# SolverForge/solverforge

Measured on AMD Instinct MI355X. Metric: moves-evaluated/sec, CVRP-1000 (nearby-list selector, LateAcceptance(400)+AcceptedCount(256)), higher is better.
Workload: dtype int64 score / int32 trial deltas (u16 matrix copy)

## Files before the change

solverforge_amd/csrc/sf_list_wave.hip:

```cpp
#pragma once
#include <hip/hip_runtime.h>
#include <stdint.h>

#include <type_traits>

#include "sf_list_model.h"

namespace sf {

constexpr uint32_t RC_MAX = 128;
constexpr uint32_t RC_SMALL = 64;
constexpr uint32_t NBR_NODE_MASK = 0x7FFFu;
constexpr uint32_t NBR_SAME_FLAG = 0x8000u;
constexpr uint32_t NBR_END = 0xFFFFu;
#ifndef SF_WPB
#define SF_WPB 4
#endif
constexpr int WPB = SF_WPB;

#ifndef SF_SPEC_V
#define SF_SPEC_V(x) (x)
#endif
#ifndef SF_SPEC_DIM
#define SF_SPEC_DIM(x) (x)
#endif
#ifndef SF_SPEC_NCAP
#define SF_SPEC_NCAP(x) (x)
#endif
#ifndef SF_SPEC_K0
#define SF_SPEC_K0(x) (x)
#endif
#ifndef SF_SPEC_K1
#define SF_SPEC_K1(x) (x)
#endif
#ifndef SF_SPEC_LA_SIZE
#define SF_SPEC_LA_SIZE(x) (x)
#endif
#ifndef SF_SPEC_LIMIT
#define SF_SPEC_LIMIT(x) (x)
#endif
#ifndef SF_SPEC_HAS_PERM
#define SF_SPEC_HAS_PERM(x) (x)
#endif
#ifndef SF_SPEC_HAS_EXPLICIT
#define SF_SPEC_HAS_EXPLICIT(x) (x)
#endif
#ifdef SF_SPEC_L
#define SF_SPEC_OWN_LANE(v) asm volatile("" : "+v"(v))
#else
#define SF_SPEC_OWN_LANE(v)
#endif
#ifdef SF_SPEC_NO_WIDE
#define SF_SPEC_WIDE_TIES(x) false
#else
#define SF_SPEC_WIDE_TIES(x) (x)
#endif
#ifdef SF_SPEC_NO_TIES
#define SF_SPEC_TIES(x) 0ULL
#else
#define SF_SPEC_TIES(x) (x)
#endif
#ifdef SF_SPEC_ROWS_FULL
#define SF_SPEC_ROW_HAVE(x) true
#define SF_SPEC_ROW_HAVEMASK(x) (~0ULL)
#else
#define SF_SPEC_ROW_HAVE(x) (x)
#define SF_SPEC_ROW_HAVEMASK(x) (x)
#endif


__device__ __forceinline__ void wave_sync() {
    __builtin_amdgcn_fence(__ATOMIC_RELEASE, "wavefront");
    __builtin_amdgcn_wave_barrier();
    __builtin_amdgcn_fence(__ATOMIC_ACQUIRE, "wavefront");
}

SF_PLAIN_KERNEL
__global__ __launch_bounds__(256) void k_nbr_presort(const int64_t* __restrict__ mat, int dim, int P,
                                                     uint16_t* __restrict__ keys) {
    extern __shared__ __attribute__((aligned(16))) unsigned char smem[];
    uint64_t* sk = (uint64_t*)smem;
    const int row = blockIdx.x;
    const int64_t* rp = mat + (size_t)row * dim;
    for (int t = threadIdx.x; t < P; t += blockDim.x) {
        uint64_t k = ~0ULL;
        if (t < dim) {
            const int64_t v = rp[t];
            if (v >= 0 && v != UNREACHABLE) k = ((uint64_t)v << 24) | (uint64_t)(uint32_t)t;
        }
        sk[t] = k;
    }
    __syncthreads();
    for (int size = 2; size <= P; size <<= 1)
        for (int stride = size >> 1; stride > 0; stride >>= 1) {
            for (int t = threadIdx.x; t < (P >> 1); t += blockDim.x) {
                const int lo = (t / stride) * 2 * stride + (t % stride);
                const int hi = lo + stride;
                const bool up = (lo & size) == 0;
                const uint64_t a = sk[lo], b = sk[hi];
                if ((a > b) == up) {
                    sk[lo] = b;
                    sk[hi] = a;
                }
            }
            __syncthreads();
        }
    for (int t = threadIdx.x; t < dim; t += blockDim.x) {
        const uint64_t k = sk[t];
        uint32_t e = NBR_END;
        if (k != ~0ULL) {
            e = (uint32_t)k & NBR_NODE_MASK;
            if (t > 0 && (sk[t - 1] >> 24) == (k >> 24)) e |= NBR_SAME_FLAG;
        }
        keys[(size_t)row * dim + t] = (uint16_t)e;
    }
}

struct WCarve {
    size_t load, off, node, ring, visits, rtab, routeat, total;
    uint32_t rc;
    __host__ __device__ WCarve(int V, int n_cap, int dim, int max_k, bool compact = false, bool node_global = false) {
        rc = max_k <= 32 ? RC_SMALL : RC_MAX;
        size_t o = 0;
        load = o;
        o = align_up(o + (compact ? sizeof(int32_t) : sizeof(int64_t)) * V, 16);
        off = o;
        o = align_up(o + (node_global ? sizeof(uint16_t) : sizeof(uint32_t)) * (V + 1), 16);
        node = o;
        o = align_up(o + (node_global ? 0 : (compact ? sizeof(uint16_t) : sizeof(uint32_t)) * dim), 16);
        ring = o;
        o = align_up(o + sizeof(uint32_t) * 2 * rc * MAX_LEAVES, 16);
        visits = o;
        o = align_up(o + sizeof(uint16_t) * n_cap, 16);
        rtab = o;
        o = align_up(o + (node_global ? 0 : sizeof(uint32_t) * V * MAX_LEAVES), 16);
        routeat = o;
        o = align_up(o + (compact ? 0 : sizeof(uint16_t) * V * MAX_LEAVES), 16);
        total = o;
    }
};

template <bool COMPACT>
struct NodeSlotT;
template <>
struct NodeSlotT<false> {
    uint32_t* p;
    __device__ __forceinline__ NodeSlotT(unsigned char* base, int, const uint16_t*, const void*, bool = false) : p((uint32_t*)base) {}
    __device__ __forceinline__ void clear(uint32_t node) const { p[node] = NODE_NONE; }
    __device__ __forceinline__ void set(uint32_t node, uint32_t route, uint32_t pos) const { p[node] = (route << 16) | pos; }
    __device__ __forceinline__ uint32_t get(uint32_t node) const { return p[node]; }
    __device__ __forceinline__ uint32_t word(uint32_t node) const { return p[node]; }
    __device__ __forceinline__ uint32_t wide(uint32_t s, uint32_t) const { return s; }
    __device__ __forceinline__ uint32_t wide_short(uint32_t s) const { return s; }
};
template <>
struct NodeSlotT<true> {
    uint16_t* p;
    const uint16_t* visits;
    const void* off;
    bool off16;
    uint32_t pb, pmax;
    __device__ __forceinline__ uint32_t off_at(uint32_t i) const { return off16 ? (uint32_t)((const uint16_t*)off)[i] : ((const uint32_t*)off)[i]; }
    __device__ __forceinline__ NodeSlotT(unsigned char* base, int V, const uint16_t* visits_, const void* off_, bool off16_ = false)
        : p((uint16_t*)base), visits(visits_), off(off_), off16(off16_) {
        uint32_t rb = 1;
        while ((1u << rb) - 1u < (uint32_t)V) ++rb;
        pb = 16u - rb;
        pmax = (1u << pb) - 1u;
    }
    __device__ __forceinline__ void clear(uint32_t node) const { p[node] = 0xFFFFu; }
    __device__ __forceinline__ void set(uint32_t node, uint32_t route, uint32_t pos) const {
        p[node] = (uint16_t)((route << pb) | (pos < pmax ? pos : pmax));
    }
    __device__ __forceinline__ uint32_t get(uint32_t node) const { return wide(p[node], node); }
    __device__ __forceinline__ uint32_t word(uint32_t node) const { return p[node]; }
    __device__ __forceinline__ uint32_t wide(uint32_t s, uint32_t node) const {
        const bool none = s == 0xFFFFu;
        const uint32_t route = s >> pb;
        uint32_t pos = s & pmax;
        if (__ballot(!none && pos == pmax) != 0ull) {
            if (!none && pos == pmax) {
                const uint32_t o = off_at(route), len = off_at(route + 1) - o;
                while (pos + 1 < len && (uint32_t)visits[o + pos] != node) ++pos;
            }
        }
        return none ? NODE_NONE : ((route << 16) | pos);
    }
    __device__ __forceinline__ uint32_t wide_short(uint32_t s) const {
        const uint32_t w = ((s >> pb) << 16) | (s & pmax);
        return s == 0xFFFFu ? NODE_NONE : w;
    }
};
__host__ __device__ inline bool node_slot_compact_ok(int V) { return V >= 1 && V <= 1022; }

struct NearbyItem {
    uint32_t w;
    uint32_t ord;
    uint32_t pay0;
    uint32_t pay1;
};

__device__ __forceinline__ NearbyItem nearby_item(bool is_change, uint32_t slot, uint32_t se, uint32_t sp,
                                                  uint32_t len, uint32_t k, const uint32_t* s_off,
                                                  const uint16_t* sb, const uint16_t* ro) {
    const bool some = slot != NODE_NONE;
    const uint32_t r2 = some ? slot >> 16 : 0u, dp = slot & 0xFFFFu;
    const uint32_t len2 = s_off[r2 + 1] - s_off[r2];
    const uint32_t rk = ro[r2];
    const uint32_t inter_ord = ORD_INTER_BASE + (uint32_t)sb[rk] + dp;
    const bool intra = r2 == se;
    const uint32_t end_pay = (r2 << 16) | len2;
    NearbyItem it;
    if (is_change) {
        const bool v0 = !intra || (dp != sp && dp != sp + 1);
        const bool v1 = dp + 1 == len2 && (!intra || len != sp + 1);
        it.w = some ? (uint32_t)v0 + (uint32_t)v1 : 0u;
        it.ord = intra ? (v0 ? dp : len) : inter_ord;
        it.pay0 = v0 ? slot : end_pay;
        it.pay1 = end_pay;
    } else {
        const bool v = intra ? dp > sp : rk > k;
        it.w = (some && v) ? 1u : 0u;
        it.ord = intra ? dp : inter_ord;
        it.pay0 = slot;
        it.pay1 = 0;
    }
    return it;
}

struct RouteTab {
    const uint32_t* rt;
    static constexpr int KEY_SHIFT = 24;
    __device__ __forceinline__ uint32_t word(uint32_t route) const { return rt[route]; }
    __device__ __forceinline__ static uint32_t rank(uint32_t w) { return w & 0xFFFFu; }
    __device__ __forceinline__ static uint32_t inter_ord(uint32_t w, uint32_t dp) { return ORD_INTER_BASE + (w >> 16) + dp; }
};
#ifdef SF_SPEC_TIE_KEY
static_assert(SF_SPEC_RB >= 1 && SF_SPEC_PB >= 1 && SF_SPEC_RB + SF_SPEC_PB <= 22, "SF_SPEC_TIE_KEY: the packed word does not fit 32 bits");
constexpr uint32_t ORD_ARITH_BASE = 1u << (SF_SPEC_RB + SF_SPEC_PB);
constexpr int ORD_ARITH_SHIFT = SF_SPEC_PB;
#else
constexpr uint32_t ORD_ARITH_BASE = 1u << 26;
constexpr int ORD_ARITH_SHIFT = 16;
#endif
struct RouteArith {
    uint32_t st, inv, V, recip;
    static constexpr int KEY_SHIFT = 28;
    __device__ __forceinline__ uint32_t word(uint32_t route) const {
        uint32_t x = route + V - st;
        x = x >= V ? x - V : x;
        const uint32_t y = x * inv;
        uint32_t rk = y - __umulhi(y, recip) * V;
        return rk >= V ? rk - V : rk;
    }
    __device__ __forceinline__ static uint32_t rank(uint32_t w) { return w; }
    __device__ __forceinline__ static uint32_t inter_ord(uint32_t w, uint32_t dp) { return ORD_ARITH_BASE + (w << ORD_ARITH_SHIFT) + dp; }
};
struct RouteRank {
    const uint32_t* rt;
    static constexpr int KEY_SHIFT = RouteArith::KEY_SHIFT;
    __device__ __forceinline__ uint32_t word(uint32_t route) const { return rt[route]; }
    __device__ __forceinline__ static uint32_t rank(uint32_t w) { return w; }
    __device__ __forceinline__ static uint32_t inter_ord(uint32_t w, uint32_t dp) { return RouteArith::inter_ord(w, dp); }
};
template <class OT, class RT>
__device__ __forceinline__ NearbyItem nearby_item_rt(bool is_change, uint32_t slot, uint32_t se, uint32_t sp,
                                                     uint32_t len, uint32_t k, const OT* s_off, const RT& rt) {
    const bool some = slot != NODE_NONE;
    const uint32_t r2 = some ? slot >> 16 : 0u, dp = slot & 0xFFFFu;
    const uint32_t len2 = s_off[r2 + 1] - s_off[r2];
    const uint32_t t = rt.word(r2);
    const uint32_t rk = RT::rank(t);
    const uint32_t inter_ord = RT::inter_ord(t, dp);
    const bool intra = r2 == se;
    const uint32_t end_pay = (r2 << 16) | len2;
    NearbyItem it;
    if (is_change) {
        const bool v0 = !intra || (dp != sp && dp != sp + 1);
        const bool v1 = dp + 1 == len2 && (!intra || len != sp + 1);
        it.w = some ? (uint32_t)v0 + (uint32_t)v1 : 0u;
        it.ord = intra ? (v0 ? dp : len) : inter_ord;
        it.pay0 = v0 ? slot : end_pay;
        it.pay1 = end_pay;
    } else {
        const bool v = intra ? dp > sp : rk > k;
        it.w = (some && v) ? 1u : 0u;
        it.ord = intra ? dp : inter_ord;
        it.pay0 = slot;
        it.pay1 = 0;
    }
    return it;
}

__device__ __forceinline__ uint32_t mbcnt64(uint64_t mask) {
    return __builtin_amdgcn_mbcnt_hi((uint32_t)(mask >> 32), __builtin_amdgcn_mbcnt_lo((uint32_t)mask, 0u));
}
#ifdef SF_SPEC_TIE_KEY
__device__ __forceinline__ int32_t tie_key_fix(uint64_t startmask, uint64_t nonstart, uint32_t ord, uint32_t wc) {
    const uint32_t q = (mbcnt64(startmask >> 1) << (SF_SPEC_RB + SF_SPEC_PB + 3)) | (ord << 2) | wc;
    uint32_t q_dn = q, q_up = q;
    int32_t fix = 0;
    uint64_t run = nonstart;
    for (uint32_t d = 1; run != 0; ++d) {
        q_dn = (uint32_t)__builtin_amdgcn_update_dpp(0, (int)q_dn, 0x130, 0xf, 0xf, true);
        q_up = (uint32_t)__builtin_amdgcn_update_dpp(0, (int)q_up, 0x138, 0xf, 0xf, true);
        fix += q_dn < q ? (int32_t)(q_dn & 3u) : 0;
        fix -= q_up > q ? (int32_t)(q_up & 3u) : 0;
        run &= nonstart << d;
    }
    return fix;
}
#endif

template <class LT, class OT, bool OWN_LANE = false>
__device__ __forceinline__ void apply_list_move_wave(const ListModel& m, uint16_t* visits, OT* off,
                                                     LT* load, int kind, uint32_t a, uint32_t i, uint32_t b,
                                                     uint32_t j, uint32_t ext = 0) {
    uint32_t lane = threadIdx.x & 63u;
    if constexpr (OWN_LANE) asm volatile("" : "+v"(lane));
    if (kind == 2) {
        const uint32_t P = off[a] + i, Q = off[b] + j;
        const uint32_t x = visits[P];
        wave_sync();
        if (P < Q) {
            for (uint32_t t0 = P; t0 < Q; t0 += 64) {
                const uint32_t t = t0 + lane;
                uint32_t nv = 0;
                if (t < Q) nv = (t + 1 < Q) ? (uint32_t)visits[t + 1] : x;
                wave_sync();
                if (t < Q) visits[t] = (uint16_t)nv;
                wave_sync();
            }
        } else if (P > Q) {
            for (uint32_t c0 = 0; c0 <= P - Q; c0 += 64) {
                const uint32_t dd = c0 + lane;
                const bool in = dd <= P - Q;
                const uint32_t t = P - (in ? dd : 0u);
                uint32_t nv = 0;
                if (in) nv = t > Q ? (uint32_t)visits[t - 1] : x;
                wave_sync();
                if (in) visits[t] = (uint16_t)nv;
                wave_sync();
            }
        }
        if (a != b) {
            for (uint32_t rr = lane; rr <= (uint32_t)SF_SPEC_V(m.V); rr += 64) {
                if (a < b && rr > a && rr <= b) off[rr] -= 1;
                if (a > b && rr > b && rr <= a) off[rr] += 1;
            }
            if (lane == 0 && m.demand) {
                const int64_t dx = (int64_t)m.demand[x];
                load[a] = (LT)wsub(load[a], dx);
                load[b] = (LT)wadd(load[b], dx);
            }
        }
    } else if (kind == 6) {
        const uint32_t za = ext & 0xFFFFu, zb = ext >> 16;
        const uint32_t PA = off[a] + i, PB = off[b] + j;
        const bool a_first = PA < PB;
        const uint32_t PX = a_first ? PA : PB, zx = a_first ? za : zb, PY = a_first ? PB : PA, zy = a_first ? zb : za;
        const uint32_t ox = a_first ? a : b, oy = a_first ? b : a;
        int64_t da = 0, db = 0;
        if (a != b && m.demand) {
            for (uint32_t t = 0; t < za; ++t) da = wadd(da, (int64_t)m.demand[visits[PA + t]]);
            for (uint32_t t = 0; t < zb; ++t) db = wadd(db, (int64_t)m.demand[visits[PB + t]]);
        }
        wave_sync();
        relocate_flat_segment(visits, PY, zy, PX, lane, 64u, [] { wave_sync(); });
        relocate_flat_segment(visits, PX + zy, zx, PY + zy, lane, 64u, [] { wave_sync(); });
        if (a != b) {
            for (uint32_t rr = lane; rr <= (uint32_t)SF_SPEC_V(m.V); rr += 64)
                if (rr > ox && rr <= oy) off[rr] = off[rr] + zy - zx;
            if (lane == 0 && m.demand) {
                load[a] = (LT)wadd(wsub(load[a], da), db);
                load[b] = (LT)wadd(wsub(load[b], db), da);
            }
        }
    } else if (kind == 5) {
        const uint32_t z = ext - i, P = off[a] + i;
        const uint32_t Q = a != b ? off[b] + j : (j <= i ? off[a] + j : off[a] + j + z);
        int64_t dsum = 0;
        if (a != b && m.demand)
            for (uint32_t t = 0; t < z; ++t) dsum = wadd(dsum, (int64_t)m.demand[visits[P + t]]);
        wave_sync();
        relocate_flat_segment(visits, P, z, Q, lane, 64u, [] { wave_sync(); });
        if (a != b) {
            for (uint32_t rr = lane; rr <= (uint32_t)SF_SPEC_V(m.V); rr += 64) {
                if (a < b && rr > a && rr <= b) off[rr] -= z;
                if (a > b && rr > b && rr <= a) off[rr] += z;
            }
            if (lane == 0 && m.demand) {
                load[a] = (LT)wsub(load[a], dsum);
                load[b] = (LT)wadd(load[b], dsum);
            }
        }
    } else if (kind == 4) {
        const uint32_t lo = off[a] + i, hi = off[a] + j;
        for (uint32_t t = lane; t < (hi - lo) / 2; t += 64) {
            const uint16_t x = visits[lo + t], y = visits[hi - 1 - t];
            visits[lo + t] = y;
            visits[hi - 1 - t] = x;
        }
    } else if (kind == 9) {
        const uint32_t base = off[a] + i, size = j - i;
        const uint32_t perm = nth_permutation_nibbles(size, ext);
        uint32_t nv = 0;
        if (lane < size) nv = visits[base + ((perm >> (4u * lane)) & 15u)];
        wave_sync();
        if (lane < size) visits[base + lane] = (uint16_t)nv;
    } else if (kind == 7) {
        const uint32_t base = off[a], c1 = i, c2 = b, c3 = j;
        const uint32_t mask = kopt_reverse_mask(ext);
        const bool rb = (mask >> 1) & 1u, rc = (mask >> 2) & 1u;
        auto reverse_range = [&](uint32_t lo, uint32_t hi) {
            for (uint32_t t = lane; t < (hi - lo) / 2; t += 64) {
                const uint16_t x = visits[base + lo + t], y = visits[base + hi - 1 - t];
                visits[base + lo + t] = y;
                visits[base + hi - 1 - t] = x;
            }
            wave_sync();
        };
        if (!kopt_swaps_segments(ext)) {
            if (rb) reverse_range(c1, c2);
            if (rc) reverse_range(c2, c3);
        } else {
            const uint32_t zc = c3 - c2;
            reverse_range(c1, c3);
            if (!rc) reverse_range(c1, c1 + zc);
            if (!rb) reverse_range(c1 + zc, c3);
        }
    } else if (kind == 3) {
        if (lane == 0) {
            const uint32_t pa = off[a] + i, pb = off[b] + j;
            const uint16_t x = visits[pa], y = visits[pb];
            visits[pa] = y;
            visits[pb] = x;
            if (a != b && m.demand) {
                const int64_t dx = (int64_t)m.demand[x], dy = (int64_t)m.demand[y];
                load[a] = (LT)wadd(wsub(load[a], dx), dy);
                load[b] = (LT)wadd(wsub(load[b], dy), dx);
            }
        }
    }
    wave_sync();
}

__device__ __forceinline__ uint32_t nearby_source_to_ring(const ListModel& m, const NbrIndex& nb, bool is_change, uint32_t se,
                                                          uint32_t sp, uint32_t len, uint32_t k, uint32_t sx,
                                                          const uint32_t* node_slot, const uint32_t* s_off, const uint16_t* sb,
                                                          const uint16_t* ro, uint32_t* rq, uint32_t RCM, uint32_t tl,
                                                          uint32_t key, uint32_t base, uint32_t need, uint32_t emitted) {
    const uint32_t lane = threadIdx.x & 63u;
    const uint64_t lanebit = 1ULL << lane;
    const uint32_t dim = (uint32_t)m.dim;
    const uint16_t* rowk = nb.keys + (size_t)sx * dim;
    const uint32_t mv0 = (se << 16) | sp;
    for (;;) {
        const bool have = key != NBR_END;
        const uint64_t havemask = __ballot(have);
        if (havemask == 0) break;
        NearbyItem it{0u, 0u, 0u, 0u};
        if (have) it = nearby_item(is_change, node_slot[key & NBR_NODE_MASK], se, sp, len, k, s_off, sb, ro);
        const uint64_t startmask = __ballot(have && (lane == 0 || !(key & NBR_SAME_FLAG)));
        const bool more = havemask == ~0ULL && base + 64 < dim;
        const uint32_t fo = 63u - (uint32_t)__clzll((unsigned long long)startmask);
        if (more && fo == 0) {
            TopK tk{~0ULL, 0u, ~0ULL};
            for (uint32_t b2 = base; b2 < dim; b2 += 64) {
                const uint32_t j2 = b2 + lane;
                const uint32_t ky = j2 < dim ? (uint32_t)rowk[j2] : NBR_END;
                NearbyItem i2{0u, 0u, 0u, 0u};
                uint64_t hk = 0;
                if (ky != NBR_END) {
                    const uint32_t y2 = ky & NBR_NODE_MASK;
                    i2 = nearby_item(is_change, node_slot[y2], se, sp, len, k, s_off, sb, ro);
                    hk = (uint64_t)m.mat[(size_t)sx * dim + y2] << 24;
                }
                if (!__ballot(ky != NBR_END)) break;
                topk_offer(tk, need, i2.w >= 1 ? (hk | i2.ord) : ~0ULL, i2.pay0);
                topk_offer(tk, need, i2.w == 2 ? (hk | (i2.ord + 1)) : ~0ULL, i2.pay1);
            }
            const uint32_t cnt = (uint32_t)__popcll(__ballot(lane < need && tk.key != ~0ULL));
            if (lane < cnt) {
                const uint32_t qi = (tl + emitted + lane) & RCM;
                rq[qi * 2] = mv0;
                rq[qi * 2 + 1] = tk.pay;
            }
            emitted += cnt;
            break;
        }
        const uint32_t nclosed = more ? fo : (uint32_t)__popcll(havemask);
        const uint64_t closedmask = nclosed >= 64 ? ~0ULL : ((1ULL << nclosed) - 1ULL);
        const bool closed = (closedmask & lanebit) != 0;
        const uint32_t wc = closed ? it.w : 0u;
        const uint64_t w1 = __ballot(wc == 1), w2 = __ballot(wc == 2);
        const uint32_t Wc = (uint32_t)__popcll(w1) + 2u * (uint32_t)__popcll(w2);
        if (Wc > 0) {
            int32_t pos = (int32_t)(mbcnt64(w1) + 2u * mbcnt64(w2));
            const uint64_t nonstart = ~startmask & closedmask;
            if (nonstart) {
                const uint32_t packed = (it.ord << 2) | wc;
                uint64_t run = nonstart;
                for (uint32_t d = 1; run != 0; ++d) {
                    const uint32_t p_dn = __shfl_down(packed, d), p_up = __shfl_up(packed, d);
                    const bool same_up = (run & lanebit) != 0;
                    const bool same_dn = ((run >> d) & lanebit) != 0;
                    if (same_dn && (p_dn >> 2) < it.ord) pos += (int32_t)(p_dn & 3u);
                    if (same_up && (p_up >> 2) > it.ord) pos -= (int32_t)(p_up & 3u);
                    run &= nonstart << d;
                }
            }
            if (wc >= 1 && (uint32_t)pos < need) {
                const uint32_t qi = (tl + emitted + (uint32_t)pos) & RCM;
                rq[qi * 2] = mv0;
                rq[qi * 2 + 1] = it.pay0;
            }
            if (wc == 2 && (uint32_t)pos + 1 < need) {
                const uint32_t qi = (tl + emitted + (uint32_t)pos + 1) & RCM;
                rq[qi * 2] = mv0;
                rq[qi * 2 + 1] = it.pay1;
            }
            const uint32_t ne = Wc < need ? Wc : need;
            emitted += ne;
            need -= ne;
        }
        if (need == 0 || !more) break;
        base += nclosed;
        const uint32_t jj = base + lane;
        key = jj < dim ? (uint32_t)rowk[jj] : NBR_END;
    }
    return emitted;
}

#if defined(SF_PHASE_PROFILE) || defined(SF_GEN_COUNT)
__device__ unsigned long long g_phase[8];
#endif
#ifdef SF_ISA_MARK
#define ISA_MARK(name) asm volatile("; SF_MARK " name)
#else
#define ISA_MARK(name)
#endif
#if defined(SF_PHASE_PROFILE) && !defined(SF_PHASE_PGRP)
#define PH_DECL uint64_t ph_t = clock64(), ph_acc[8] = {0, 0, 0, 0, 0, 0, 0, 0};
#define PH(i)                          \
    {                                  \
        const uint64_t _t = clock64(); \
        ph_acc[i] += _t - ph_t;        \
        ph_t = _t;                     \
    }
#define PH_DUMP \
    if (lane == 0) for (int _k = 0; _k < 8; ++_k) atomicAdd(&g_phase[_k], (unsigned long long)ph_acc[_k]);
#elif defined(SF_GEN_COUNT)
#define PH_DECL uint64_t ph_acc[8] = {0, 0, 0, 0, 0, 0, 0, 0};
#define PH(i)
#define GC(i) ph_acc[i] += 1;
#define PH_DUMP \
    if (lane == 0) for (int _k = 0; _k < 8; ++_k) atomicAdd(&g_phase[_k], (unsigned long long)ph_acc[_k]);
#else
#define PH_DECL
#define PH(i)
#define PH_DUMP
#endif
#ifndef GC
#define GC(i)
#endif

__device__ __forceinline__ int32_t wave_max_i32(int32_t v) {
    const int lo = (int)0x80000000;
    v = max(v, __builtin_amdgcn_update_dpp(lo, v, 0x111, 0xf, 0xf, false));
    v = max(v, __builtin_amdgcn_update_dpp(lo, v, 0x112, 0xf, 0xf, false));
    v = max(v, __builtin_amdgcn_update_dpp(lo, v, 0x114, 0xf, 0xf, false));
    v = max(v, __builtin_amdgcn_update_dpp(lo, v, 0x118, 0xf, 0xf, false));
    v = max(v, __builtin_amdgcn_update_dpp(lo, v, 0x142, 0xa, 0xf, false));
    v = max(v, __builtin_amdgcn_update_dpp(lo, v, 0x143, 0xc, 0xf, false));
    return __builtin_amdgcn_readlane(v, 63);
}
template <int L>
__device__ __forceinline__ bool small_ge(const int32_t (&a)[L], const int32_t (&b)[L]) {
    bool ge = true;
#pragma unroll
    for (int k = L - 1; k >= 0; --k) ge = a[k] > b[k] || (a[k] == b[k] && ge);
    return ge;
}
template <int L>
__device__ __forceinline__ bool small_ge0(const int32_t (&a)[L]) {
    bool ge = true;
#pragma unroll
    for (int k = L - 1; k >= 0; --k) ge = a[k] > 0 || (a[k] == 0 && ge);
    return ge;
}
__device__ __forceinline__ int32_t clamp_i64_to_i32(int64_t v) {
    return v > 0x7FFFFFFFll ? 0x7FFFFFFF : v < -0x7FFFFFFFll - 1 ? (int32_t)0x80000000 : (int32_t)v;
}

template <int L, class LT, bool M16 = false, class OT = uint32_t>
__device__ __forceinline__ bool eval_list_move_small(const ListModel& m, const uint16_t* visits, const OT* off, const LT* load,
                                                     bool chg, uint32_t a, uint32_t i, uint32_t b, uint32_t j, int32_t (&dv)[L]) {
    const uint32_t oa = off[a], la = off[a + 1] - oa;
    const uint32_t ob = off[b], lb = off[b + 1] - ob;
    const bool intra = a == b;
    bool ok = i < la && (chg ? j <= lb : j < lb) && !(intra && (j == i || (chg && j == i + 1)));
    const bool flip = !chg && intra && i > j;
    const uint32_t i2 = ok ? (flip ? j : i) : 0u, j2 = ok ? (flip ? i : j) : 0u;
    const uint32_t la_ = ok ? la : 0u, lb_ = ok ? lb : 0u;
    const uint32_t depot = (uint32_t)m.depot;
    const uint32_t P = oa + i2, Q = ob + j2;
    const bool has_pa = i2 > 0, has_na = i2 + 1 < la_, has_q = j2 < lb_, has_pb = j2 > 0, has_nb = j2 + 1 < lb_;
    const uint32_t r_x = visits[P];
    const uint32_t x = ok ? r_x : depot;
    const uint32_t r_pa = visits[has_pa ? P - 1 : P], r_na = visits[has_na ? P + 1 : P];
    const uint32_t r_q = visits[has_q ? Q : P], r_pb = visits[has_pb ? Q - 1 : P], r_nb = visits[has_nb ? Q + 1 : P];
    const uint32_t pa = has_pa ? r_pa : depot, na = has_na ? r_na : depot;
    const uint32_t vq = has_q ? r_q : depot;
    const uint32_t pb = has_pb ? r_pb : depot, nb = has_nb ? r_nb : depot;
    ok = ok && (chg || x != vq);
    const bool adj = !chg && intra && j2 == i2 + 1;
    const bool ca = chg || adj;
    const bool src_single = la == 1, dst_empty = !intra && lb == 0;
    const uint32_t dim4 = (uint32_t)SF_SPEC_DIM(m.dim) * (M16 ? 2u : 4u);
    auto leg = [&](uint32_t f, uint32_t t) -> uint32_t {
        const uint32_t byte_off = f * dim4 + t * (M16 ? 2u : 4u);
        if (M16) return *(const uint16_t*)((const char*)m.mat16 + byte_off);
        return *(const uint32_t*)((const char*)m.mat32 + byte_off);
    };
    const uint32_t p0 = leg(pa, chg ? na : vq);
    const uint32_t p1 = leg(chg ? pb : vq, ca ? x : na);
    const uint32_t p2 = leg(ca ? x : pb, chg ? vq : (adj ? nb : x));
    const uint32_t p3 = leg(x, nb);
    const uint32_t m0 = leg(pa, x);
    const uint32_t m1 = leg(x, adj ? vq : na);
    const uint32_t m3 = leg(vq, nb);
    const uint32_t m2 = leg(adj ? vq : pb, adj ? nb : vq);
    int32_t d_cap = 0;
    if (m.cap_level >= 0) {
        const int32_t dx = m.demand[x];
        const int32_t dyq = m.demand[vq];
        const int32_t dy = chg ? 0 : dyq;
        const int32_t cap = (int32_t)m.capacity;
        const int32_t la0 = (int32_t)load[a], lb0 = (int32_t)load[b];
        const int32_t la1 = la0 - dx + dy, lb1 = lb0 - dy + dx;
        d_cap = max(la1 - cap, 0) + max(lb1 - cap, 0) - max(la0 - cap, 0) - max(lb0 - cap, 0);
        d_cap = intra ? 0 : d_cap;
    }
    const uint32_t plus = ((chg && src_single) ? 0u : p0) + p1 + p2 + (ca ? 0u : p3);
    const uint32_t minus = m0 + m1 + ((chg && dst_empty) ? 0u : m2) + (ca ? 0u : m3);
    const int32_t d_dist = (int32_t)(plus - minus);
    const int32_t cw = (int32_t)m.cap_weight, dw = (int32_t)m.dist_weight;
#pragma unroll
    for (int k = 0; k < L; ++k) {
        int32_t v = 0;
        if (k == m.cap_level) v -= cw * d_cap;
        if (k == m.dist_level) v -= dw * d_dist;
        dv[k] = ok ? v : 0;
    }
    return ok;
}

template <int L>
struct LevelWords {
    uint32_t wc[L], wd[L];
    uint32_t has_cap;
    int32_t cap, cw, dw;
    uint32_t depot;
};
template <int L, bool USED, bool KW>
__device__ __forceinline__ LevelWords<L> level_words(const ListModel& m) {
    LevelWords<L> w;
    w.cap = w.cw = w.dw = 0;
    w.depot = 0;
#ifdef SF_SPEC_MODEL_WORDS
    w.cap = SF_SPEC_CAPACITY, w.cw = SF_SPEC_CAP_WEIGHT, w.dw = SF_SPEC_DIST_WEIGHT, w.depot = SF_SPEC_DEPOT;
#pragma unroll
    for (int k = 0; k < L; ++k) w.wc[k] = k == SF_SPEC_CAP_LEVEL ? 0xFFFFFFFFu : 0u, w.wd[k] = k == SF_SPEC_DIST_LEVEL ? 0xFFFFFFFFu : 0u;
    w.has_cap = SF_SPEC_CAP_LEVEL >= 0 ? 1u : 0u;
    return w;
#endif
    if constexpr (KW) {
        auto word = [](uint32_t v) -> uint32_t {
            asm volatile("" : "+v"(v));
            return uni(v);
        };
        w.cap = (int32_t)word((uint32_t)m.capacity);
        w.cw = (int32_t)word((uint32_t)m.cap_weight);
        w.dw = (int32_t)word((uint32_t)m.dist_weight);
        w.depot = word((uint32_t)m.depot);
    }
#pragma unroll
    for (int k = 0; k < L; ++k) {
        w.wc[k] = uni(k == m.cap_level ? 0xFFFFFFFFu : 0u);
        w.wd[k] = uni(k == m.dist_level ? 0xFFFFFFFFu : 0u);
        if constexpr (USED) {
            asm volatile("" : "+s"(w.wc[k]));
            asm volatile("" : "+s"(w.wd[k]));
        }
    }
    w.has_cap = uni(m.cap_level >= 0 ? 1u : 0u);
    if constexpr (USED) asm volatile("" : "+s"(w.has_cap));
    return w;
}
template <int L, class LT, bool M16 = false, class OT = uint32_t, bool KW = false>
__device__ __forceinline__ void eval_generated_small(const ListModel& m, const LevelWords<L>& lw, const uint16_t* visits, const OT* off, const LT* load, uint32_t c,
                                                     uint32_t a, uint32_t i, uint32_t b, uint32_t j, int32_t (&dv)[L]) {
    const uint32_t oa = off[a], la = off[a + 1] - oa;
    const uint32_t ob = off[b], lb = off[b + 1] - ob;
    const uint32_t depot = KW ? lw.depot : (uint32_t)m.depot;
    const uint32_t P = oa + i, Q = ob + j;
    const uint32_t h_pa = min(i, 1u), h_na = min(la - 1u - i, 1u);
    const uint32_t h_q = min(lb - j, 1u), h_pb = min(j, 1u);
    const uint32_t h_nb = min(max(lb, j + 1u) - (j + 1u), 1u);
    const uint32_t x = visits[P];
    const uint32_t r_pa = visits[P - h_pa], r_na = visits[P + h_na];
    const uint32_t r_q = visits[Q - (1u - h_q)], r_pb = visits[Q - h_pb], r_nb = visits[Q + h_nb];
    const uint32_t pa = h_pa ? r_pa : depot, na = h_na ? r_na : depot;
    const uint32_t vq = h_q ? r_q : depot;
    const uint32_t pb = h_pb ? r_pb : depot, nb = h_nb ? r_nb : depot;
    const bool chg = c != 0;
    const bool intra = a == b;
    const bool adj = !chg && intra && j == i + 1;
    const bool ca = chg || adj;
    const uint32_t dim4 = (uint32_t)SF_SPEC_DIM(m.dim) * (M16 ? 2u : 4u);
    auto leg = [&](uint32_t f, uint32_t t) -> uint32_t {
        const uint32_t byte_off = __umul24(f, dim4) + t * (M16 ? 2u : 4u);
        if (M16) return *(const uint16_t*)((const char*)m.mat16 + byte_off);
        return *(const uint32_t*)((const char*)m.mat32 + byte_off);
    };
    const uint32_t p0 = leg(pa, chg ? na : vq);
    const uint32_t p1 = leg(chg ? pb : vq, ca ? x : na);
    const uint32_t p2 = leg(ca ? x : pb, chg ? vq : (adj ? nb : x));
    const uint32_t p3 = leg(x, nb);
    const uint32_t m0 = leg(pa, x);
    const uint32_t m1 = leg(x, adj ? vq : na);
    const uint32_t m3 = leg(vq, nb);
    const uint32_t m2 = leg(adj ? vq : pb, adj ? nb : vq);
    int32_t d_cap = 0;
    if (lw.has_cap != 0u) {
        const int32_t dx = m.demand[x];
        const int32_t dyq = m.demand[vq];
        const int32_t dy = chg ? 0 : dyq;
        const int32_t cap = KW ? lw.cap : (int32_t)m.capacity;
        const int32_t la0 = (int32_t)load[a] - cap, lb0 = (int32_t)load[b] - cap;
        const int32_t sh = dx - dy;
        d_cap = max(la0 - sh, 0) + max(lb0 + sh, 0) - max(la0, 0) - max(lb0, 0);
        d_cap = intra ? 0 : d_cap;
    }
    const uint32_t plus = ((chg && la == 1) ? 0u : p0) + p1 + p2 + (ca ? 0u : p3);
    const uint32_t minus = m0 + m1 + ((chg && !intra && lb == 0) ? 0u : m2) + (ca ? 0u : m3);
    const int32_t d_dist = (int32_t)(plus - minus);
    const int32_t tc = -((KW ? lw.cw : (int32_t)m.cap_weight) * d_cap), td = -((KW ? lw.dw : (int32_t)m.dist_weight) * d_dist);
#pragma unroll
    for (int k = 0; k < L; ++k) dv[k] = (int32_t)(((uint32_t)tc & lw.wc[k]) + ((uint32_t)td & lw.wd[k]));
}

struct LeafCursor {
    uint32_t head, tail;
    uint32_t left;
    uint32_t k, o;
    uint32_t se, len, sp, sx;
    uint32_t vk, vbase;
    int ex;
    uint32_t pk;
    uint32_t pv;
    uint32_t cend;
};

struct WaveArgs {
    ListModel m;
    SearchParams p;
    NbrIndex nb;
};
typedef const __attribute__((address_space(4))) WaveArgs* ColdArgs;
__device__ __forceinline__ ColdArgs cold_args() {
    uint64_t u = (uint64_t)__builtin_amdgcn_kernarg_segment_ptr();
    asm volatile("" : "+s"(u));
    return (ColdArgs)u;
}

#ifndef SF_WAVES_PER_EU
#define SF_WAVES_PER_EU 4
#endif
template <int L, bool TRACE, int MODE, bool COMPACT = false, int WPE = SF_WAVES_PER_EU, bool NODEG = false>
__global__ __launch_bounds__(64 * WPB, WPE) void k_list_search_wave(ListModel m, SearchParams p, NbrIndex nb) {
    constexpr bool FAST = MODE >= 1, SMALL = MODE == 2;
    constexpr bool LEAN = FAST && SMALL;
    constexpr bool SAT = LEAN && COMPACT, RANKTAB = LEAN && COMPACT && !NODEG;
    constexpr bool RBATCH = LEAN && !NODEG;
#define SF_COLD_P(f) (SMALL ? cold_args()->p.f : p.f)
#define SF_COLD_M(f) (SMALL ? cold_args()->m.f : m.f)
    static_assert(!COMPACT || SMALL, "COMPACT stores loads in 32 bits: MODE 2 only");
    static_assert(!NODEG || COMPACT, "NODEG: the 16-bit table of the COMPACT layout");
    using LT = typename std::conditional<COMPACT, int32_t, int64_t>::type;
    using OT = typename std::conditional<NODEG, uint16_t, uint32_t>::type;
    extern __shared__ __attribute__((aligned(16))) unsigned char smem[];
    const uint32_t lane = threadIdx.x & 63u;
    const uint32_t wave_in_group = uni(threadIdx.x >> 6);
    const int rr = (int)(blockIdx.x * (blockDim.x >> 6) + wave_in_group);
    if (rr >= p.n_launch) return;
    const int r = rr + p.replica_base;
    const int V = SF_SPEC_V(m.V);
    const uint32_t dim = (uint32_t)SF_SPEC_DIM(m.dim);

    const int n_leaves = FAST ? 2 : p.n_leaves;
    const uint32_t K0 = (uint32_t)SF_SPEC_K0(p.leaf[0].max_nearby), K1 = n_leaves > 1 ? (uint32_t)SF_SPEC_K1(p.leaf[1].max_nearby) : 1u;
    const bool chg0 = FAST ? true : p.leaf[0].kind == 16, chg1 = FAST ? false : (n_leaves > 1 && p.leaf[1].kind == 16);
    const int acceptor = FAST ? 1 : p.acceptor, forager = FAST ? 0 : p.forager;
    const bool dry_run = FAST ? false : p.dry_run != 0;
    __shared__ uint64_t s_sa[FAST ? 1 : WPB][FAST ? 1 : SA_WORDS];
    uint64_t* saw = s_sa[FAST ? 0 : wave_in_group];
    const bool annealing = !FAST && acceptor == 3;
    if constexpr (!FAST)
        if (annealing) sa_load(saw, p.sa, r, lane);
    const int32_t desc0_w = p.leaf[0].descriptor, desc1_w = n_leaves > 1 ? p.leaf[1].descriptor : 0;
    const uint64_t desc0_q = SMALL ? 0 : (uint64_t)p.leaf[0].descriptor, desc1_q = (!SMALL && n_leaves > 1) ? (uint64_t)p.leaf[1].descriptor : 0;
    auto desc0 = [&]() -> uint64_t { return SMALL ? (uint64_t)(int64_t)desc0_w : desc0_q; };
    auto desc1 = [&]() -> uint64_t { return SMALL ? (uint64_t)(int64_t)desc1_w : desc1_q; };

    const WCarve cv(V, SF_SPEC_NCAP(m.n_cap), (int)dim, (int)(K0 > K1 ? K0 : K1), COMPACT, NODEG);
    const uint32_t RCM = cv.rc - 1;
    unsigned char* mem = smem + (size_t)wave_in_group * cv.total;
    LT* s_load = (LT*)(mem + cv.load);
    OT* s_off = (OT*)(mem + cv.off);
    uint32_t* ring = (uint32_t*)(mem + cv.ring);
    uint16_t* s_visits = (uint16_t*)(mem + cv.visits);
    const NodeSlotT<COMPACT> node_slot(NODEG ? (unsigned char*)(m.node_tab + (size_t)r * dim) : mem + cv.node, V, s_visits, (const void*)s_off, NODEG);
    auto node_sync = [&]() {
        if constexpr (NODEG) {
            __builtin_amdgcn_fence(__ATOMIC_RELEASE, "workgroup");
            __builtin_amdgcn_wave_barrier();
            __builtin_amdgcn_fence(__ATOMIC_ACQUIRE, "workgroup");
        } else {
            wave_sync();
        }
    };
    constexpr bool ARANK = NODEG;
    using RT = typename std::conditional<ARANK, RouteArith, typename std::conditional<RANKTAB, RouteRank, RouteTab>::type>::type;
    uint32_t* rtab = (uint32_t*)(mem + cv.rtab);
    uint16_t* route_at = (uint16_t*)(mem + cv.routeat);

    uint32_t* g_visits = m.visits + (size_t)r * SF_SPEC_NCAP(m.n_cap);
    uint32_t* g_off = m.off + (size_t)r * (V + 1);
    int64_t* g_load = m.load + (size_t)r * V;
    int64_t* g_score = m.score + (size_t)r * 4;
    const bool tracing = TRACE && r == p.trace_replica;

    for (uint32_t t = lane; t <= (uint32_t)V; t += 64) s_off[t] = (OT)g_off[t];
    for (uint32_t t = lane; t < (uint32_t)V; t += 64) s_load[t] = (LT)g_load[t];
    for (uint32_t t = lane; t < dim; t += 64) node_slot.clear(t);
    node_sync();
    const uint32_t total0 = uni(s_off[V]);
    if (COMPACT && SF_SPEC_HAS_PERM(m.perm != nullptr)) {
        for (uint32_t t = lane; t < total0; t += 64) s_visits[t] = m.perm[g_visits[t]];
    } else {
        for (uint32_t t = lane; t < total0; t += 64) s_visits[t] = (uint16_t)g_visits[t];
    }
    wave_sync();
    for (uint32_t v = lane; v < (uint32_t)V; v += 64) {
        const uint32_t o = s_off[v], len = s_off[v + 1] - o;
        for (uint32_t q = 0; q < len; ++q) node_slot.set(s_visits[o + q], v, q);
    }
    node_sync();

    uint32_t nsat = 0;
    if constexpr (SAT) {
        for (uint32_t base = 0; base < (uint32_t)V; base += 64) {
            const uint32_t v = base + lane;
            const bool lg = v < (uint32_t)V && (uint32_t)(s_off[v + 1] - s_off[v]) > node_slot.pmax;
            nsat += (uint32_t)__popcll(__ballot(lg));
        }
    }
    auto ext_id = [&](uint32_t x) -> uint32_t { return (COMPACT && SF_SPEC_HAS_PERM(m.inv != nullptr)) ? (uint32_t)m.inv[x] : x; };
    int64_t cur[L], best_sol[L];
#pragma unroll
    for (int k = 0; k < L; ++k) {
        cur[k] = (int64_t)uni64((uint64_t)g_score[k]);
        best_sol[k] = (int64_t)uni64((uint64_t)m.best_score[(size_t)r * 4 + k]);
    }
    uint32_t st_steps = 0, st_gen = 0, st_acc = 0, st_applied = 0, st_calc = 0, st_scored = 0, st_sources = 0;
    uint64_t steps_run = 0;
    auto flush_stats = [&]() {
        if (lane == 0) {
            uint64_t* gs = SF_COLD_P(stats) + (size_t)r * SF_STATS_WORDS;
            gs[0] += st_steps;
            gs[1] += st_gen;
            gs[2] += st_gen;
            gs[3] += st_acc;
            gs[4] += st_applied;
            gs[5] += st_calc;
            gs[6] += st_gen - st_calc;
            gs[7] += st_scored;
            gs[8] += st_sources;
        }
        if constexpr (!SMALL) steps_run += st_steps;
        st_steps = st_gen = st_acc = st_applied = st_calc = st_scored = st_sources = 0;
    };
    uint64_t trace_n = 0;
    const uint64_t step_index0 = dry_run ? 0 : p.step_index[r];
    const uint64_t seed_draws0 = dry_run ? 0 : p.seed_draws[r];
    const int la_idx0 = dry_run ? 0 : p.la_idx[r];
    int la_cursor = la_idx0;
    const uint64_t lanebit = 1ULL << lane;
    uint32_t hm = 0;
    if constexpr (LEAN) {
        hm = (uint32_t)((int32_t)(lane << 26) >> 31);
        asm volatile("" : "+v"(hm));
    }
    auto half = [&](uint32_t lo, uint32_t up) -> uint32_t { return (lo & ~hm) | (up & hm); };
    PH_DECL

    const LevelWords<L> lvl = level_words<L, SMALL, RBATCH>(m);
    bool best_pending = false;
    const FastMod fm_V = make_fastmod(V > 0 ? (uint32_t)V : 1u);
    const FastMod fm_V1 = make_fastmod(V > 1 ? (uint32_t)V - 1u : 1u);
    const uint32_t v_recip32 = V > 1 ? (uint32_t)(0x100000000ull / (uint32_t)V) : 0u;
    const bool use_cm = V >= 2 && V <= 128;
    const uint64_t cm_lo = use_cm ? __ballot(lane >= 1 && lane < (uint32_t)V && gcd_u32(lane, (uint32_t)V) == 1) : 0ull;
    const uint64_t cm_hi = use_cm ? __ballot(lane + 64 < (uint32_t)V && gcd_u32(lane + 64, (uint32_t)V) == 1) : 0ull;
    int64_t step = 0;
    for (; step < SF_COLD_P(n_steps); ++step) {
        PH(7)
        ISA_MARK("prologue_begin");
        uint64_t sidx, sseed;
        if (dry_run) {
            sidx = p.dry_step_index;
            sseed = p.dry_step_seed;
        } else {
            sidx = step_index0 + (uint64_t)step;
            const uint64_t draw = seed_draws0 + (uint64_t)step;
            const uint64_t* const explicit_seeds = SF_COLD_P(explicit_seeds);
            const int64_t n_explicit = SF_COLD_P(n_explicit);
            if (SF_SPEC_HAS_EXPLICIT(explicit_seeds != nullptr) && (int64_t)draw < n_explicit)
                sseed = explicit_seeds[(size_t)r * n_explicit + draw];
            else
                sseed = step_seed(SF_COLD_P(random_seed) + (uint64_t)r, draw);
        }
        sidx = uni64(sidx);
        sseed = uni64(sseed);
        const StreamCtx ctx{sidx, sseed, FAST ? 3 : p.order};
        ScoreV<L> late;
#pragma unroll
        for (int k = 0; k < L; ++k) late.v[k] = 0;
        const int la_slot = la_cursor;
        if (acceptor == 1 || acceptor == 4) {
            const int64_t* const lh = SF_COLD_P(la_hist) + ((size_t)r * SF_SPEC_LA_SIZE(SF_COLD_P(la_size)) + la_slot) * 4;
#pragma unroll
            for (int k = 0; k < L; ++k) late.v[k] = (int64_t)uni64((uint64_t)lh[k]);
        }
        ScoreV<L> dla_thr = late;
        if (acceptor == 4) {
            ScoreV<L> db;
#pragma unroll
            for (int k = 0; k < L; ++k) db.v[k] = (int64_t)uni64((uint64_t)p.dla_best[(size_t)r * 4 + k]);
            dla_thr = dla_threshold<L>(db, p.dla_tolerance);
        }
        [[maybe_unused]] bool thr_on = true;
        if constexpr (TRACE)
            if (acceptor == 5 || acceptor == 6) ax_step_begin<L>(acceptor, p.sa.state + (size_t)r * SA_WORDS, late, thr_on);
        [[maybe_unused]] TabuStep<L> tabu;
        [[maybe_unused]] const TabuScope tabu_scope{0u, 0u, 0u};
        if constexpr (TRACE)
            if (acceptor == 7) tabu_step_begin<L>(p.sa.state + (size_t)r * SA_WORDS, tabu);
        int has_best = 0;
        typename std::conditional<SMALL, uint32_t, uint64_t>::type equal_count = 0;
        uint32_t accepted = 0, pulls = 0;
        ScoreV<L> best;
#pragma unroll
        for (int k = 0; k < L; ++k) best.v[k] = 0;
        uint32_t best_m0 = 0, best_m1 = 0;
        int best_leaf = 0;
        uint64_t best_ti = 0;
        int32_t late_d[L], best_d[L];
#pragma unroll
        for (int k = 0; k < L; ++k) {
            late_d[k] = SMALL ? clamp_i64_to_i32(wsub(late.v[k], cur[k])) : 0;
            best_d[k] = 0;
        }
        int64_t acc_thr = 0, best_key = 0;
        if constexpr (SMALL && L == 2) {
            const int64_t lh = late_d[0] < -(1 << 30) ? -(int64_t)(1 << 30) : (int64_t)late_d[0];
            const int64_t late_key = lh * 4294967296ll + (int64_t)late_d[1];
            acc_thr = late_key < 0 ? late_key : 0;
        }
        const uint32_t total = uni(s_off[V]);
        uint32_t hashed = 0;
        const bool lane_hash = FAST && use_cm;
        if (lane_hash) {
            const uint64_t es0 = SALT_NEARBY_CHANGE_ENTITY ^ desc0(), es1 = SALT_NEARBY_SWAP_ENTITY ^ desc1();
            const uint64_t salt = lane == 0 ? SALT_UNION_OFFSET : lane == 1 ? es0 : lane == 2 ? (es0 ^ STRIDE_SALT_MIX) : lane == 3 ? es1 : (es1 ^ STRIDE_SALT_MIX);
            const FastMod fm2 = make_fastmod(2u);
            FastMod f;
            f.M = lane == 0 ? fm2.M : ((lane & 1u) ? fm_V.M : fm_V1.M);
            f.n = lane == 0 ? fm2.n : ((lane & 1u) ? fm_V.n : fm_V1.n);
            hashed = fastmod_u64(ctx.mixed_seed(salt), f);
        }
        const uint32_t first_leaf = lane_hash ? (uint32_t)__builtin_amdgcn_readlane((int)hashed, 0)
                                              : (n_leaves > 1 ? ctx.random_index((uint32_t)n_leaves, SALT_UNION_OFFSET) : 0u);

        uint32_t perm_st0 = 0, perm_sd0 = 1, perm_st1 = 0, perm_sd1 = 1;
        uint32_t perm_inv0 = 0, perm_inv1 = 0;
        auto route_facts = [&](int l) -> RT {
            if constexpr (ARANK)
                return RouteArith{l ? perm_st1 : perm_st0, l ? perm_inv1 : perm_inv0, (uint32_t)V, v_recip32};
            else
                return RT{rtab + l * V};
        };
        auto resolve = [&](LeafCursor& c, int l) {
            const uint16_t* ra = route_at + l * V;
            uint32_t k = c.k, o = c.o, se = c.se, len = c.len;
            if (o >= c.cend) {
            ISA_MARK("resolve_slow_begin");
            if (k != c.vk || o >= len) {
                for (;;) {
                    if constexpr (COMPACT) {
                        const uint32_t xx = (l ? perm_st1 : perm_st0) + k * (l ? perm_sd1 : perm_sd0);
                        uint32_t rr_ = xx - __umulhi(xx, v_recip32) * (uint32_t)V;
                        rr_ = rr_ >= (uint32_t)V ? rr_ - (uint32_t)V : rr_;
                        se = uni(rr_);
                    } else
                        se = uni((uint32_t)ra[k]);
                    len = uni(s_off[se + 1] - s_off[se]);
                    if (o < len) break;
                    ++k;
                    o = 0;
                }
            }
            if (k != c.vk || (o & ~63u) != c.vbase) {
                const uint64_t src_salt = ((l ? chg1 : chg0) ? SALT_NEARBY_CHANGE_SOURCE : SALT_NEARBY_SWAP_SOURCE) ^
                                          (uint64_t)se ^ (l ? desc1() : desc0());
                const uint32_t oo = (o & ~63u) + lane;
                const uint32_t spl = oo < len ? ctx.selection_index(oo, len, src_salt) : 0u;
                const uint32_t sxl = oo < len ? (uint32_t)s_visits[s_off[se] + spl] : 0u;
                c.pv = spl | (sxl << 16);
                c.vk = k;
                c.vbase = o & ~63u;
            }
            c.cend = len < (o & ~63u) + 64u ? len : (o & ~63u) + 64u;
            c.k = k;
            c.se = se;
            c.len = len;
            ISA_MARK("resolve_slow_end");
            }
            const uint32_t pvv = (uint32_t)__builtin_amdgcn_readlane((int)c.pv, (int)(o & 63u));
            const uint32_t sp = pvv & 0xFFFFu, sx = pvv >> 16;
            c.o = o;
            c.sp = sp;
            c.sx = sx;
            const uint32_t ent = l ? ((lane + 32u) & 63u) : lane;
            const uint32_t entc = ent < dim ? ent : dim - 1u;
            const uint32_t pk_any = (uint32_t) * (const uint16_t*)((const char*)nb.keys + ((sx * dim + entc) << 1));
            if constexpr (LEAN)
                c.pk = pk_any;
            else
                c.pk = ent < dim ? pk_any : NBR_END;
        };
        auto row_key = [&](uint32_t raw, uint32_t e) -> uint32_t { return LEAN ? (e < dim ? raw : NBR_END) : raw; };

        PH(0)
        LeafCursor C0{0, 0, total, 0, 0, 0, 0, 0, 0, 0xFFFFFFFFu, 0, 0, NBR_END, 0, 0};
        LeafCursor C1{0, 0, n_leaves > 1 ? total : 0u, 0, 0, 0, 0, 0, 0, 0xFFFFFFFFu, 0, n_leaves > 1 ? 0 : 1, NBR_END, 0, 0};
        for (int l = 0; l < n_leaves; ++l) {
            const uint64_t ent_salt = ((l ? chg1 : chg0) ? SALT_NEARBY_CHANGE_ENTITY : SALT_NEARBY_SWAP_ENTITY) ^ (l ? desc1() : desc0());
            uint32_t pst, psd;
            if (lane_hash) {
                pst = (uint32_t)__builtin_amdgcn_readlane((int)hashed, l ? 3 : 1);
                psd = StreamCtx::first_coprime_from((uint32_t)__builtin_amdgcn_readlane((int)hashed, l ? 4 : 2) + 1u, cm_lo, cm_hi);
            } else if (use_cm)
                ctx.perm_params_fm(fm_V, fm_V1, ent_salt, pst, psd, cm_lo, cm_hi);
            else
                ctx.perm_params((uint32_t)V, ent_salt, pst, psd);
            pst = uni(pst);
            psd = uni(psd);
            if (l)
                perm_st1 = pst, perm_sd1 = psd;
            else
                perm_st0 = pst, perm_sd0 = psd;
            if constexpr (ARANK) {
                uint32_t inv = 0;
                for (uint32_t base = 0; base < (uint32_t)V; base += 64) {
                    const uint32_t c = base + lane;
                    const uint32_t xx = psd * c;
                    uint32_t rm = xx - __umulhi(xx, v_recip32) * (uint32_t)V;
                    rm = rm >= (uint32_t)V ? rm - (uint32_t)V : rm;
                    const uint64_t hit = __ballot(c < (uint32_t)V && rm == 1u);
                    if (hit) {
                        inv = base + (uint32_t)__ffsll((unsigned long long)hit) - 1u;
                        break;
                    }
                }
                if (l)
                    perm_inv1 = inv;
                else
                    perm_inv0 = inv;
                continue;
            }
            uint16_t* ra = route_at + l * V;
            uint32_t* rt = rtab + l * V;
            [[maybe_unused]] uint32_t carry = 0;
            for (uint32_t base = 0; base < (uint32_t)V; base += 64) {
                const uint32_t k = base + lane;
                if constexpr (RANKTAB) {
                    if (k < (uint32_t)V) rt[perm_index_recip(pst, psd, k, (uint32_t)V, v_recip32)] = k;
                } else {
                    uint32_t v = 0, e = 0;
                    if (k < (uint32_t)V) {
                        e = fastmod_u64((uint64_t)pst + (uint64_t)k * psd, fm_V);
                        if constexpr (!COMPACT) ra[k] = (uint16_t)e;
                        v = s_off[e + 1] - s_off[e] + 1;
                    }
                    const uint32_t inc = wave_incl_scan(v);
                    if (k < (uint32_t)V) rt[e] = k | ((carry + inc - v) << 16);
                    carry += __shfl(inc, 63);
                }
            }
        }
        wave_sync();
        if constexpr (SMALL) st_sources += C0.left + C1.left;
        if (total > 0) {
            resolve(C0, 0);
            if (n_leaves > 1) resolve(C1, 1);
        }
        ISA_MARK("prologue_end");

        PH(1)
        int done = 0;
        while (!done) {
            PH(4)
            auto gen_rest = [&](int l, uint32_t se, uint32_t sp, uint32_t len, uint32_t k, uint32_t sx, uint32_t tl,
                                uint32_t key, uint32_t base, uint32_t need, uint32_t emitted) -> uint32_t {
                const bool is_change = l ? chg1 : chg0;
                const RT rt = route_facts(l);
                uint32_t* rq = ring + (size_t)l * cv.rc * 2;
                const uint16_t* rowk = nb.keys + (size_t)sx * dim;
                const uint32_t mv0 = (se << 16) | sp;
                for (;;) {
                    const bool have = key != NBR_END;
                    const uint64_t havemask = __ballot(have);
                    if (havemask == 0) break;
                    NearbyItem it{0u, 0u, 0u, 0u};
                    if (have) it = nearby_item_rt(is_change, node_slot.get(key & NBR_NODE_MASK), se, sp, len, k, s_off, rt);
                    const uint64_t startmask = __ballot(have && (lane == 0 || !(key & NBR_SAME_FLAG)));
                    const bool more = havemask == ~0ULL && base + 64 < dim;
                    const uint32_t fo = 63u - (uint32_t)__clzll((unsigned long long)startmask);
                    if (SF_SPEC_WIDE_TIES(more && fo == 0)) {
                        TopK tk{~0ULL, 0u, ~0ULL};
                        for (uint32_t b2 = base; b2 < dim; b2 += 64) {
                            const uint32_t j2 = b2 + lane;
                            const uint32_t ky = j2 < dim ? (uint32_t)rowk[j2] : NBR_END;
                            NearbyItem i2{0u, 0u, 0u, 0u};
                            uint64_t hk = 0;
                            if (ky != NBR_END) {
                                const uint32_t y2 = ky & NBR_NODE_MASK;
                                i2 = nearby_item_rt(is_change, node_slot.get(y2), se, sp, len, k, s_off, rt);
                                hk = (uint64_t)m.mat[(size_t)ext_id(sx) * dim + ext_id(y2)] << RT::KEY_SHIFT;
                            }
                            if (!__ballot(ky != NBR_END)) break;
                            topk_offer(tk, need, i2.w >= 1 ? (hk | i2.ord) : ~0ULL, i2.pay0);
                            topk_offer(tk, need, i2.w == 2 ? (hk | (i2.ord + 1)) : ~0ULL, i2.pay1);
                        }
                        const uint32_t cnt = (uint32_t)__popcll(__ballot(lane < need && tk.key != ~0ULL));
                        if (lane < cnt) {
                            const uint32_t qi = (tl + emitted + lane) & RCM;
                            rq[qi * 2] = mv0;
                            rq[qi * 2 + 1] = tk.pay;
                        }
                        emitted += cnt;
                        break;
                    }
                    const uint32_t nclosed = more ? fo : (uint32_t)__popcll(havemask);
                    const uint64_t closedmask = nclosed >= 64 ? ~0ULL : ((1ULL << nclosed) - 1ULL);
                    const bool closed = (closedmask & lanebit) != 0;
                    const uint32_t wc = closed ? it.w : 0u;
                    const uint64_t w1 = __ballot(wc == 1), w2 = __ballot(wc == 2);
                    const uint32_t Wc = (uint32_t)__popcll(w1) + 2u * (uint32_t)__popcll(w2);
                    GC(l ? 6 : 5)
                    if (Wc == 0) { GC(7) }
                    if (Wc > 0) {
                        int32_t pos = (int32_t)(mbcnt64(w1) + 2u * mbcnt64(w2));
                        const uint64_t nonstart = SF_SPEC_TIES(~startmask & closedmask);
#ifdef SF_SPEC_TIE_KEY
                        if (nonstart) pos += tie_key_fix(startmask, nonstart, it.ord, wc);
#else
                        if (nonstart) {
                            const uint32_t packed = (it.ord << 2) | wc;
                            uint64_t run = nonstart;
                            uint32_t p_dn = packed, p_up = packed;
                            for (uint32_t d = 1; run != 0; ++d) {
                                p_dn = (uint32_t)__builtin_amdgcn_update_dpp(0, (int)p_dn, 0x130, 0xf, 0xf, false);
                                p_up = (uint32_t)__builtin_amdgcn_update_dpp(0, (int)p_up, 0x138, 0xf, 0xf, false);
                                const bool same_up = (run & lanebit) != 0;
                                const bool same_dn = ((run >> d) & lanebit) != 0;
                                if (same_dn && (p_dn >> 2) < it.ord) pos += (int32_t)(p_dn & 3u);
                                if (same_up && (p_up >> 2) > it.ord) pos -= (int32_t)(p_up & 3u);
                                run &= nonstart << d;
                            }
                        }
#endif
                        if (wc >= 1 && (uint32_t)pos < need) {
                            const uint32_t qi = (tl + emitted + (uint32_t)pos) & RCM;
                            rq[qi * 2] = mv0;
                            rq[qi * 2 + 1] = it.pay0;
                        }
                        if (wc == 2 && (uint32_t)pos + 1 < need) {
                            const uint32_t qi = (tl + emitted + (uint32_t)pos + 1) & RCM;
                            rq[qi * 2] = mv0;
                            rq[qi * 2 + 1] = it.pay1;
                        }
                        const uint32_t ne = Wc < need ? Wc : need;
                        emitted += ne;
                        need -= ne;
                    }
                    if (need == 0 || !more) break;
                    base += nclosed;
                    const uint32_t jj = base + lane;
                    key = jj < dim ? (uint32_t)rowk[jj] : NBR_END;
                }
                return emitted;
            };
            auto slot_of = [&](uint32_t word, uint32_t node) -> uint32_t {
                if constexpr (SAT) {
                    uint32_t ns = nsat;
                    asm volatile("" : "+s"(ns));
                    if (ns != 0) return node_slot.wide(word, node);
                    return node_slot.wide_short(word);
                } else
                    return node_slot.wide(word, node);
            };
            const uint32_t single0 = cv.rc - K0 < 64u ? cv.rc - K0 : 64u, single1 = cv.rc - K1 < 64u ? cv.rc - K1 : 64u;
            ISA_MARK("fill_begin");
            for (;;) {
                const bool both_live = !C0.ex && !C1.ex;
                const bool need0 = !C0.ex && C0.left > 0 && C0.tail - C0.head < (both_live ? 32u : single0);
                const bool need1 = n_leaves > 1 && !C1.ex && C1.left > 0 && C1.tail - C1.head < (both_live ? 32u : single1);
                if (!need0 && !need1) break;
                if (need0 && need1) {
                    ISA_MARK("pair_begin");
                    GC(0)
                    const bool hi = lane >= 32;
                    const uint32_t seA = C0.se, spA = C0.sp, lenA = C0.len, kA = C0.k, sxA = C0.sx, tlA = C0.tail;
                    const uint32_t seB = C1.se, spB = C1.sp, lenB = C1.len, kB = C1.k, sxB = C1.sx, tlB = C1.tail;
                    uint32_t l31 = lane & 31u;
                    if constexpr (LEAN) asm volatile("" : "+v"(l31));
                    const uint32_t key = LEAN ? (SF_SPEC_ROW_HAVE(false) ? half(C0.pk, C1.pk) : row_key(half(C0.pk, C1.pk), l31)) : (hi ? C1.pk : C0.pk);
                    const bool have = SF_SPEC_ROW_HAVE(key != NBR_END);
                    uint32_t nd = have ? (key & NBR_NODE_MASK) : 0u;
                    uint32_t slot_word = 0;
                    if constexpr (LEAN) {
                        asm volatile("" : "+v"(nd)::"memory");
                        slot_word = node_slot.word(nd);
                    }
                    C0.left -= 1;
                    C0.o += 1;
                    if (C0.left > 0) resolve(C0, 0);
                    C1.left -= 1;
                    C1.o += 1;
                    if (C1.left > 0) resolve(C1, 1);
                    if constexpr (!SMALL) st_sources += 2;
                    uint32_t slot_any;
                    if constexpr (LEAN)
                        slot_any = slot_of(slot_word, nd);
                    else
                        slot_any = node_slot.get(nd);
                    const uint32_t slot = have ? slot_any : NODE_NONE;
                    NearbyItem it{0u, 0u, 0u, 0u};
                    uint32_t mv0, tl, Kh, rq_off;
                    if constexpr (LEAN) {
                        const uint32_t sev = half(seA, seB), spv = half(spA, spB);
                        mv0 = (sev << 16) | spv;
                        tl = half(tlA, tlB);
                        Kh = half(K0, K1);
                        rq_off = hm & (cv.rc * 2u);
                        const bool some = slot != NODE_NONE;
                        const uint32_t r_any = slot >> 16, dp = slot & 0xFFFFu;
                        const uint32_t r2 = some ? r_any : 0u;
                        const uint32_t len2 = s_off[r2 + 1] - s_off[r2];
                        uint32_t t;
                        if constexpr (ARANK)
                            t = RouteArith{half(perm_st0, perm_st1), half(perm_inv0, perm_inv1), (uint32_t)V, v_recip32}.word(r2);
                        else
                            t = rtab[r2 + (hm & (uint32_t)V)];
                        const bool intra = r2 == sev;
                        const uint32_t end_pay = (r2 << 16) | len2;
                        const uint32_t xi = dp - (spv & ~hm), yi = half(1u, spv);
                        const uint32_t xo = RT::rank(t) | ~hm, yo = kB & hm;
                        const uint32_t xs = intra ? xi : xo, ys = intra ? yi : yo;
                        const bool v0 = xs > ys;
                        const uint32_t last = lenA ^ (spv + 1u);
                        const uint32_t f = intra ? last : 1u;
                        const uint32_t z1 = (((dp + 1u) ^ len2) | hm) | (1u - min(f, 1u));
                        const bool v1 = z1 == 0u;
                        const uint32_t b0 = v0 ? 1u : 0u, b1 = v1 ? 1u : 0u;
                        const uint32_t wsum = b0 + b1;
                        it.w = some ? wsum : 0u;
                        const uint32_t len_or_dp = half(lenA, dp), ord_intra = v0 ? dp : len_or_dp, ord_inter = RT::inter_ord(t, dp);
                        it.ord = intra ? ord_intra : ord_inter;
                        const uint32_t end_or_slot = half(end_pay, slot);
                        it.pay0 = v0 ? slot : end_or_slot;
                        it.pay1 = end_pay;
                    } else {
                        const uint32_t se = hi ? seB : seA, sp = hi ? spB : spA, len = hi ? lenB : lenA, kk = hi ? kB : kA;
                        mv0 = (se << 16) | sp;
                        tl = hi ? tlB : tlA;
                        Kh = hi ? K1 : K0;
                        rq_off = hi ? cv.rc * 2u : 0u;
                        RT rth;
                        if constexpr (ARANK)
                            rth = RouteArith{hi ? perm_st1 : perm_st0, hi ? perm_inv1 : perm_inv0, (uint32_t)V, v_recip32};
                        else
                            rth = RT{rtab + (hi ? V : 0)};
                        if constexpr (FAST) {
                            const bool some = slot != NODE_NONE;
                            const uint32_t r2 = some ? slot >> 16 : 0u, dp = slot & 0xFFFFu;
                            const uint32_t len2 = s_off[r2 + 1] - s_off[r2];
                            const uint32_t t = rth.word(r2);
                            const bool intra = r2 == se;
                            const uint32_t end_pay = (r2 << 16) | len2;
                            const bool v0 = hi ? (intra ? dp > sp : RT::rank(t) > kk) : (!intra || dp - sp >= 2u);
                            const bool v1 = !hi && dp + 1 == len2 && (!intra || len != sp + 1);
                            it.w = some ? (uint32_t)v0 + (uint32_t)v1 : 0u;
                            it.ord = intra ? ((hi || v0) ? dp : len) : RT::inter_ord(t, dp);
                            it.pay0 = (hi || v0) ? slot : end_pay;
                            it.pay1 = end_pay;
                        } else {
                            const NearbyItem ic = nearby_item_rt(true, slot, se, sp, len, kk, s_off, rth);
                            const NearbyItem is = nearby_item_rt(false, slot, se, sp, len, kk, s_off, rth);
                            const bool lane_change = hi ? chg1 : chg0;
                            it.w = lane_change ? ic.w : is.w;
                            it.ord = lane_change ? ic.ord : is.ord;
                            it.pay0 = lane_change ? ic.pay0 : is.pay0;
                            it.pay1 = lane_change ? ic.pay1 : is.pay1;
                        }
                    }
                    const uint64_t havemask = SF_SPEC_ROW_HAVEMASK(__ballot(have));
                    const uint64_t startmask = LEAN ? __ballot(key < NBR_END - min(l31, 1u) * (NBR_END - NBR_SAME_FLAG))
                                                        : __ballot(have && (l31 == 0 || !(key & NBR_SAME_FLAG)));
                    const uint32_t hvA = (uint32_t)havemask, hvB = (uint32_t)(havemask >> 32);
                    const uint32_t stA = (uint32_t)startmask, stB = (uint32_t)(startmask >> 32);
                    const bool moreA = hvA == 0xFFFFFFFFu && 32u < dim, moreB = hvB == 0xFFFFFFFFu && 32u < dim;
                    uint32_t ncA = 0, ncB = 0;
                    uint64_t closedmask;
                    bool closed;
                    if constexpr (LEAN) {
                        const uint32_t hvv = half(hvA, hvB), stv = half(stA, stB);
                        const uint32_t ncv = (hvv == 0xFFFFFFFFu && 32u < dim) ? 31u - (uint32_t)__clz(stv) : (uint32_t)__popc(hvv);
                        closed = l31 < ncv;
                        closedmask = __ballot(closed);
                    } else {
                        ncA = moreA ? 31u - (uint32_t)__clz(stA) : (uint32_t)__popc(hvA);
                        ncB = moreB ? 31u - (uint32_t)__clz(stB) : (uint32_t)__popc(hvB);
                        closedmask = (uint64_t)(ncA >= 32 ? 0xFFFFFFFFu : ((1u << ncA) - 1u)) |
                                     ((uint64_t)(ncB >= 32 ? 0xFFFFFFFFu : ((1u << ncB) - 1u)) << 32);
                        closed = (closedmask & lanebit) != 0;
                    }
                    const uint32_t wc = closed ? it.w : 0u;
                    const uint64_t w1 = __ballot(wc == 1), w2 = __ballot(wc == 2);
                    const uint32_t WcA = (uint32_t)__popc((uint32_t)w1) + 2u * (uint32_t)__popc((uint32_t)w2);
                    const uint32_t WcB = (uint32_t)__popc((uint32_t)(w1 >> 32)) + 2u * (uint32_t)__popc((uint32_t)(w2 >> 32));
                    if (WcA + WcB > 0) {
                        const uint32_t pa = __builtin_amdgcn_mbcnt_lo((uint32_t)w1, 0u) + 2u * __builtin_amdgcn_mbcnt_lo((uint32_t)w2, 0u);
                        const uint32_t pb = __builtin_amdgcn_mbcnt_hi((uint32_t)(w1 >> 32), 0u) + 2u * __builtin_amdgcn_mbcnt_hi((uint32_t)(w2 >> 32), 0u);
                        int32_t pos = (int32_t)(LEAN ? half(pa, pb) : (hi ? pb : pa));
                        const uint64_t nonstart = SF_SPEC_TIES(~startmask & closedmask);
#ifdef SF_SPEC_TIE_KEY
                        static_assert(!std::is_same<RT, RouteTab>::value, "SF_SPEC_TIE_KEY: the (rank, position) ordinals");
                        if (nonstart) pos += tie_key_fix(startmask, nonstart, it.ord, wc);
#else
                        if (nonstart) {
                            const uint32_t packed = (it.ord << 2) | wc;
                            uint64_t run = nonstart;
                            uint32_t p_dn = packed, p_up = packed;
                            for (uint32_t d = 1; run != 0; ++d) {
                                p_dn = (uint32_t)__builtin_amdgcn_update_dpp(0, (int)p_dn, 0x130, 0xf, 0xf, false);
                                p_up = (uint32_t)__builtin_amdgcn_update_dpp(0, (int)p_up, 0x138, 0xf, 0xf, false);
                                const bool same_up = (run & lanebit) != 0;
                                const bool same_dn = ((run >> d) & lanebit) != 0;
                                if (same_dn && (p_dn >> 2) < it.ord) pos += (int32_t)(p_dn & 3u);
                                if (same_up && (p_up >> 2) > it.ord) pos -= (int32_t)(p_up & 3u);
                                run &= nonstart << d;
                            }
                        }
#endif
                        uint32_t* rq = ring + rq_off;
                        if (wc >= 1 && (uint32_t)pos < Kh) {
                            const uint32_t qi = (tl + (uint32_t)pos) & RCM;
                            rq[qi * 2] = mv0;
                            rq[qi * 2 + 1] = it.pay0;
                        }
                        if (wc == 2 && (uint32_t)pos + 1 < Kh) {
                            const uint32_t qi = (tl + (uint32_t)pos + 1) & RCM;
                            rq[qi * 2] = mv0;
                            rq[qi * 2 + 1] = it.pay1;
                        }
                    }
                    uint32_t emA = WcA < K0 ? WcA : K0, emB = WcB < K1 ? WcB : K1;
                    if (emA < K0 && moreA) {
                        GC(3)
                        ISA_MARK("pair_rest_begin");
                        if constexpr (LEAN) ncA = 31u - (uint32_t)__clz(stA);
                        const uint32_t jj = ncA + lane;
                        emA = gen_rest(0, seA, spA, lenA, kA, sxA, tlA, jj < dim ? (uint32_t)nb.keys[(size_t)sxA * dim + jj] : NBR_END, ncA, K0 - emA, emA);
                        ISA_MARK("pair_rest_end");
                    }
                    if (emB < K1 && moreB) {
                        GC(4)
                        ISA_MARK("pair_rest_begin");
                        if constexpr (LEAN) ncB = 31u - (uint32_t)__clz(stB);
                        const uint32_t jj = ncB + lane;
                        emB = gen_rest(1, seB, spB, lenB, kB, sxB, tlB, jj < dim ? (uint32_t)nb.keys[(size_t)sxB * dim + jj] : NBR_END, ncB, K1 - emB, emB);
                        ISA_MARK("pair_rest_end");
                    }
                    C0.tail = tlA + emA;
                    C1.tail = tlB + emB;
                    ISA_MARK("pair_end");
                } else {
                    const int l = need0 ? 0 : 1;
                    GC(l ? 2 : 1)
                    LeafCursor c = l ? C1 : C0;
                    const uint32_t se = c.se, sp = c.sp, len = c.len, k = c.k, sx = c.sx;
                    uint32_t key = row_key(l ? __shfl(c.pk, (int)((lane + 32u) & 63u)) : c.pk, lane);
                    if constexpr (LEAN) asm volatile("" : "+v"(key)::"memory");
                    c.left -= 1;
                    c.o += 1;
                    if (c.left > 0) resolve(c, l);
                    if constexpr (!SMALL) st_sources += 1;
                    c.tail += gen_rest(l, se, sp, len, k, sx, c.tail, key, 0u, l ? K1 : K0, 0u);
                    if (l)
                        C1 = c;
                    else
                        C0 = c;
                }
            }
            ISA_MARK("fill_end");
            wave_sync();
            PH(2)

            ISA_MARK("replay_begin");
            {
                const bool live0 = !C0.ex, live1 = !C1.ex;
                if (!live0 && !live1) {
                    done = 1;
                    break;
                }
                const bool both = live0 && live1;
                uint32_t lf, idx;
                if (both) {
                    const uint32_t l0 = (first_leaf + pulls) & 1u;
                    lf = (l0 + lane) & 1u;
                    idx = (lf ? C1.head : C0.head) + (lane >> 1);
                } else {
                    lf = live0 ? 0u : 1u;
                    idx = (lf ? C1.head : C0.head) + lane;
                }
                const bool avail = (int32_t)((lf ? C1.tail : C0.tail) - idx) > 0;
                const uint64_t availmask = __ballot(avail);
                const uint32_t nvalid = availmask == ~0ULL ? 64u : (uint32_t)(__ffsll((unsigned long long)~availmask) - 1);
                if (nvalid == 0) {
                    const uint32_t lf0 = uni(__shfl(lf, 0));
                    if (lf0)
                        C1.ex = 1;
                    else
                        C0.ex = 1;
                    continue;
                }
                const bool valid = lane < nvalid;
                uint32_t m0 = 0, m1 = 0;
                ScoreV<L> sc;
#pragma unroll
                for (int kk = 0; kk < L; ++kk) sc.v[kk] = 0;
                bool doable = false, acc = false, consumed = false, improving_pick = false;
                uint64_t accmask = 0;
                uint32_t nconsumed = nvalid;
                if constexpr (SMALL) {
                    int32_t dv[L];
                    {
                        const uint32_t lf0 = (uint32_t)__builtin_amdgcn_readfirstlane((int)lf), idx0 = (uint32_t)__builtin_amdgcn_readfirstlane((int)idx);
                        const uint32_t lfq = valid ? lf : lf0;
                        const uint32_t qi = (valid ? idx : idx0) & RCM;
                        const uint32_t* rq = ring + ((size_t)lfq * cv.rc + qi) * 2;
                        m0 = rq[0];
                        m1 = rq[1];
                        const uint32_t a = m0 >> 16, i = m0 & 0xFFFFu, b = m1 >> 16, j = m1 & 0xFFFFu;
                        eval_generated_small<L, LT, COMPACT, OT, RBATCH>(m, lvl, s_visits, s_off, s_load, 1u - lfq, a, i, b, j, dv);
                    }
                    doable = valid;
                    int64_t key = 0;
                    if constexpr (L == 2) {
                        key = (int64_t)(((uint64_t)(uint32_t)dv[0] << 32) + (uint64_t)(int64_t)dv[1]);
                        acc = valid && key >= acc_thr;
                    } else {
                        acc = valid && (small_ge0<L>(dv) || small_ge<L>(dv, late_d));
                    }
                    accmask = __ballot(acc);
                    consumed = valid;
                    if (!RBATCH || (uint32_t)__popcll(accmask) >= (uint32_t)SF_SPEC_LIMIT(p.limit) - accepted) {
                        const uint32_t remaining = (uint32_t)SF_SPEC_LIMIT(p.limit) - accepted;
                        const uint32_t pre = mbcnt64(accmask) + (acc ? 1u : 0u);
                        const uint64_t cutmask = __ballot(acc && pre == remaining);
                        nconsumed = cutmask ? (uint32_t)__ffsll((unsigned long long)cutmask) : nvalid;
                        consumed = lane < nconsumed;
                        acc = acc && consumed;
                        accmask = __ballot(acc);
                        if constexpr (RBATCH) {
                            st_scored += nvalid - nconsumed;
                            done = 1;
                        }
                    }
                    bool challenger;
                    if constexpr (L == 2)
                        challenger = acc && key >= best_key;
                    else
                        challenger = acc && small_ge<L>(dv, best_d);
                    if (accmask && (!has_best || __ballot(challenger))) {
                        int32_t M[L];
                        bool in_max = acc;
#pragma unroll
                        for (int kk = 0; kk < L; ++kk) {
                            M[kk] = wave_max_i32(in_max ? dv[kk] : (int32_t)0x80000000);
                            in_max = in_max && dv[kk] == M[kk];
                        }
                        int64_t Mkey = 0;
                        if constexpr (L == 2) Mkey = (int64_t)(((uint64_t)(uint32_t)M[0] << 32) + (uint64_t)(int64_t)M[1]);
                        bool ge, gt;
                        if constexpr (L == 2) {
                            ge = !has_best || Mkey >= best_key;
                            gt = !has_best || Mkey > best_key;
                        } else {
                            ge = !has_best || small_ge<L>(M, best_d);
                            gt = !has_best || !small_ge<L>(best_d, M);
                        }
                        if (ge) {
                            const bool newmax = gt;
                            const uint32_t eq_base = newmax ? 0u : equal_count;
                            const uint64_t eq = __ballot(in_max);
                            const uint32_t rank = mbcnt64(eq) + 1u;
                            const uint64_t cntq = (uint64_t)(eq_base + rank);
                            const bool pick = in_max && ((newmax && rank == 1) ||
                                                         (p.random_ties && cntq > 1 && reservoir_pick(sseed, cntq)));
                            const uint64_t pm = __ballot(pick);
                            if (pm) {
                                const int sel = 63 - __clzll((unsigned long long)pm);
                                best_m0 = __shfl(m0, sel);
                                best_m1 = __shfl(m1, sel);
                                best_leaf = (int)__shfl(lf, sel);
                            }
                            if constexpr (L == 2) {
                                best_key = Mkey;
                            } else {
#pragma unroll
                                for (int kk = 0; kk < L; ++kk) best_d[kk] = M[kk];
                            }
                            equal_count = eq_base + (uint32_t)__popcll(eq);
                            has_best = 1;
                        }
                    }
                } else {
                    ListDelta dl{0, 0, false};
                    if (valid) {
                        const uint32_t qi = idx & RCM;
                        const uint32_t* rq = ring + ((size_t)lf * cv.rc + qi) * 2;
                        m0 = rq[0];
                        m1 = rq[1];
                        const uint32_t a = m0 >> 16, i = m0 & 0xFFFFu, b = m1 >> 16, j = m1 & 0xFFFFu;
                        dl = eval_list_move_legs<uint16_t, FAST>(m, s_visits, s_off, s_load, lf ? chg1 : chg0, a, i, b, j);
                    }
                    sc = apply_delta<L>(m, cur, dl);
                    ScoreV<L> curv;
    #pragma unroll
                    for (int kk = 0; kk < L; ++kk) curv.v[kk] = cur[kk];
                    doable = valid && dl.doable;
                    if (doable) {
                        if (acceptor == 0)
                            acc = score_cmp<L>(sc, curv) > 0;
                        else if (acceptor == 1)
                            acc = score_cmp<L>(sc, curv) >= 0 || score_cmp<L>(sc, late) >= 0;
                        else if (acceptor == 4)
                            acc = score_cmp<L>(sc, curv) >= 0 || score_cmp<L>(sc, late) >= 0 || score_cmp<L>(sc, dla_thr) >= 0;
                    }
                    if constexpr (TRACE)
                        if (acceptor == 5 || acceptor == 6) acc = ax_accepts<L>(doable, sc, curv, late, thr_on);
                    if constexpr (TRACE)
                        if (acceptor == 7) {
                            TabuSig sig{{TABU_NO_TOKEN, TABU_NO_TOKEN}, {TABU_NO_TOKEN, TABU_NO_TOKEN}, {0, 0}, {0, 0}};
                            if (doable) {
                                const uint32_t a = m0 >> 16, i = m0 & 0xFFFFu, b = m1 >> 16, j = m1 & 0xFFFFu;
                                const uint32_t u = ext_id(s_visits[s_off[a] + i]);
                                if (lf ? chg1 : chg0)
                                    tabu_sig_list_change(tabu_scope, a, i, b, (a == b && j > i) ? j - 1 : j, u, sig);
                                else
                                    tabu_sig_list_swap(tabu_scope, a, i, u, b, j, ext_id(s_visits[s_off[b] + j]), sig);
                            }
                            acc = tabu_accepts<L>(tabu, doable, sc, sig);
                        }
                    SaChunk sach;
                    if constexpr (!FAST)
                        if (annealing) acc = sa_decide<L>(saw, p.sa, doable, sc, curv, lane, sach);
                    accmask = __ballot(acc);
                    ScoreV<L> forager_thr = curv;
                    if (forager == FORAGER_FIRST_BEST_IMPROVING) {
    #pragma unroll
                        for (int kk = 0; kk < L; ++kk) forager_thr.v[kk] = best_sol[kk];
                    }
                    nconsumed = forager_chunk_cut<L>(forager, (uint32_t)SF_SPEC_LIMIT(p.limit), accepted, acc, sc, forager_thr, nvalid, improving_pick);
                    consumed = lane < nconsumed;
                    if constexpr (!FAST)
                        if (annealing) sa_commit<L>(saw, p.sa, sach, nconsumed, lane);
                    acc = acc && consumed;
                    accmask = __ballot(acc);
                    if (accmask) {
                        if (improving_pick) {
                            const int sel = (int)nconsumed - 1;
    #pragma unroll
                            for (int kk = 0; kk < L; ++kk) best.v[kk] = (int64_t)uni64(shfl_u64((uint64_t)sc.v[kk], sel));
                            best_m0 = __shfl(m0, sel);
                            best_m1 = __shfl(m1, sel);
                            best_leaf = (int)__shfl(lf, sel);
                            if (TRACE) best_ti = trace_n + (uint64_t)sel;
                            equal_count = 1;
                            has_best = 1;
                        } else if (forager == 1) {
                            if (!has_best) {
                                const int sel = __ffsll((unsigned long long)accmask) - 1;
    #pragma unroll
                                for (int kk = 0; kk < L; ++kk) best.v[kk] = (int64_t)uni64(shfl_u64((uint64_t)sc.v[kk], sel));
                                best_m0 = __shfl(m0, sel);
                                best_m1 = __shfl(m1, sel);
                                best_leaf = (int)__shfl(lf, sel);
                                if (TRACE) best_ti = trace_n + (uint64_t)sel;
                                has_best = 1;
                            }
                        } else if (!has_best || __ballot(acc && score_cmp<L>(sc, best) >= 0)) {
                            const ScoreV<L> M = wave_max_score<L>(sc, acc);
                            const int cm = has_best ? score_cmp<L>(M, best) : 1;
                            if (cm >= 0) {
                                const bool newmax = cm > 0;
                                const uint64_t eq_base = newmax ? 0 : equal_count;
                                const bool in_eq = acc && score_cmp<L>(sc, M) == 0;
                                const uint64_t eq = __ballot(in_eq);
                                const uint32_t rank = mbcnt64(eq) + 1u;
                                const uint64_t cntq = eq_base + rank;
                                const bool pick = in_eq && ((newmax && rank == 1) ||
                                                            (p.random_ties && cntq > 1 && reservoir_pick(sseed, cntq)));
                                const uint64_t pm = __ballot(pick);
                                if (pm) {
                                    const int sel = 63 - __clzll((unsigned long long)pm);
                                    best_m0 = __shfl(m0, sel);
                                    best_m1 = __shfl(m1, sel);
                                    best_leaf = (int)__shfl(lf, sel);
                                    if (TRACE) best_ti = trace_n + (uint64_t)sel;
                                }
    #pragma unroll
                                for (int kk = 0; kk < L; ++kk) best.v[kk] = (int64_t)uni64((uint64_t)M.v[kk]);
                                equal_count = eq_base + (uint64_t)__popcll(eq);
                                has_best = 1;
                            }
                        }
                    }
                }
                const uint32_t nacc = (uint32_t)__popcll(accmask);
                accepted += nacc;
                if constexpr (!RBATCH) st_scored += nvalid;
                if constexpr (!SMALL) {
                    st_gen += nconsumed;
                    st_acc += nacc;
                    const uint32_t ndo = (uint32_t)__popcll(__ballot(consumed && doable));
                    st_calc += ndo;
                }
                if (tracing && consumed) {
                    const uint64_t ti = trace_n + lane;
                    if ((int64_t)ti < p.trace_cap) {
                        int32_t* tm = p.trace_moves + ti * 6;
                        tm[0] = (lf ? chg1 : chg0) ? 2 : 3;
                        tm[1] = (int32_t)(m0 >> 16);
                        tm[2] = (int32_t)(m0 & 0xFFFFu);
                        tm[3] = (int32_t)(m1 >> 16);
                        tm[4] = (int32_t)(m1 & 0xFFFFu);
                        tm[5] = -1;
                        for (int kk = 0; kk < L && kk < m.levels; ++kk) p.trace_scores[ti * m.levels + kk] = doable ? sc.v[kk] : 0;
                        p.trace_flags[ti] = (doable ? 1 : 0) | (acc ? 2 : 0) | ((int32_t)lf << 8);
                    }
                }
                if (tracing) trace_n += nconsumed;
                uint32_t c1;
                if constexpr (SMALL) {
                    const uint32_t lfirst = (uint32_t)__builtin_amdgcn_readfirstlane((int)lf);
                    c1 = both ? ((nconsumed + lfirst) >> 1) : (lfirst ? nconsumed : 0u);
                } else {
                    c1 = (uint32_t)__popcll(__ballot(consumed && lf == 1u));
                }
                C1.head += c1;
                C0.head += nconsumed - c1;
                pulls += nconsumed;
                if constexpr (!RBATCH)
                    if (forager_quits(forager, (uint32_t)SF_SPEC_LIMIT(p.limit), accepted, has_best, improving_pick)) done = 1;
            }
            ISA_MARK("replay_end");
            PH(3)
        }
        PH(4)

        ISA_MARK("commit_begin");
        if constexpr (SMALL) st_sources -= C0.left + C1.left;
        if constexpr (SMALL) {
            if constexpr (L == 2) {
                const int32_t soft = (int32_t)(uint32_t)(uint64_t)best_key;
                best_d[1] = soft;
                best_d[0] = (int32_t)(uint32_t)((uint64_t)wsub(best_key, (int64_t)soft) >> 32);
            }
#pragma unroll
            for (int kk = 0; kk < L; ++kk) best.v[kk] = wadd(cur[kk], (int64_t)best_d[kk]);
        }
        const bool applied = has_best && !dry_run;
        [[maybe_unused]] TabuSig pick_sig;
        if (applied) {
            if (best_pending) {
                ScoreV<L> bs;
#pragma unroll
                for (int kk = 0; kk < L; ++kk) bs.v[kk] = best_sol[kk];
                if (!(score_cmp<L>(best, bs) > 0)) {
                    const uint32_t tot = uni(s_off[V]);
                    uint32_t* const bv = SF_COLD_M(best_visits) + (size_t)r * SF_SPEC_NCAP(SF_COLD_M(n_cap));
                    uint32_t* const bo = SF_COLD_M(best_off) + (size_t)r * (V + 1);
                    uint32_t ln = lane;
                    if constexpr (RANKTAB) asm volatile("" : "+v"(ln));
                    for (uint32_t t = ln; t < tot; t += 64) bv[t] = ext_id(s_visits[t]);
                    for (uint32_t t = ln; t <= (uint32_t)V; t += 64) bo[t] = s_off[t];
                    best_pending = false;
                }
            }
            const int kind = (best_leaf ? chg1 : chg0) ? 2 : 3;
            const uint32_t a = uni(best_m0 >> 16), i = uni(best_m0 & 0xFFFFu);
            const uint32_t b = uni(best_m1 >> 16), j = uni(best_m1 & 0xFFFFu);
            if (tracing && lane == 0) {
                p.trace_applied[0] = 1;
                if ((int64_t)best_ti < p.trace_cap) p.trace_flags[best_ti] |= 4;
                p.trace_applied[1] = kind;
                p.trace_applied[2] = (int32_t)a;
                p.trace_applied[3] = (int32_t)i;
                p.trace_applied[4] = (int32_t)b;
                p.trace_applied[5] = (int32_t)j;
                p.trace_applied[6] = -1;
            }
            if constexpr (SAT) {
                if (kind == 2 && a != b) {
                    const uint32_t la0 = uni(s_off[a + 1] - s_off[a]), lb0 = uni(s_off[b + 1] - s_off[b]);
                    nsat += (lb0 == node_slot.pmax ? 1u : 0u);
                    nsat -= (la0 == node_slot.pmax + 1u ? 1u : 0u);
                }
                nsat = uni(nsat);
            }
            if constexpr (TRACE)
                if (acceptor == 7) {
                    const uint32_t u = ext_id(s_visits[s_off[a] + i]);
                    if (kind == 2)
                        tabu_sig_list_change(tabu_scope, a, i, b, (a == b && j > i) ? j - 1 : j, u, pick_sig);
                    else
                        tabu_sig_list_swap(tabu_scope, a, i, u, b, j, ext_id(s_visits[s_off[b] + j]), pick_sig);
                }
            apply_list_move_wave<LT, OT, RANKTAB && L == 4>(m, s_visits, s_off, s_load, kind, a, i, b, j);
            {
                const uint32_t oa = s_off[a], la = s_off[a + 1] - oa;
                const uint32_t ob = s_off[b], lb = s_off[b + 1] - ob;
                for (uint32_t t = lane; t < la + (a != b ? lb : 0u); t += 64) {
                    if (t < la)
                        node_slot.set(s_visits[oa + t], a, t);
                    else
                        node_slot.set(s_visits[ob + (t - la)], b, t - la);
                }
            }
            node_sync();
#pragma unroll
            for (int kk = 0; kk < L; ++kk) cur[kk] = best.v[kk];
            st_applied += 1;
        } else if (tracing && lane == 0) {
            p.trace_applied[0] = 0;
        }
        if (!dry_run) {
            bool improved = false;
            if (applied) {
                ScoreV<L> cs, bs;
#pragma unroll
                for (int kk = 0; kk < L; ++kk) {
                    cs.v[kk] = cur[kk];
                    bs.v[kk] = best_sol[kk];
                }
                improved = score_cmp<L>(cs, bs) > 0;
            }
            if (improved) {
                best_pending = true;
#pragma unroll
                for (int kk = 0; kk < L; ++kk) best_sol[kk] = cur[kk];
            }
            const int la_size = SF_SPEC_LA_SIZE(SF_COLD_P(la_size));
            if ((acceptor == 1 || acceptor == 4) && lane == 0) {
                int64_t* const lh = SF_COLD_P(la_hist) + ((size_t)r * la_size + la_slot) * 4;
#pragma unroll
                for (int kk = 0; kk < L; ++kk) lh[kk] = cur[kk];
            }
            if (acceptor == 4 && lane == 0) {
                ScoreV<L> cs, db;
#pragma unroll
                for (int kk = 0; kk < L; ++kk) {
                    cs.v[kk] = cur[kk];
                    db.v[kk] = p.dla_best[(size_t)r * 4 + kk];
                }
                if (score_cmp<L>(cs, db) > 0) {
#pragma unroll
                    for (int kk = 0; kk < L; ++kk) p.dla_best[(size_t)r * 4 + kk] = cur[kk];
                }
            }
            if constexpr (TRACE)
                if (acceptor == 5 || acceptor == 6) ax_step_ended<L>(acceptor, lane == 0, cur, p.sa.state + (size_t)r * SA_WORDS);
            if constexpr (TRACE)
                if (acceptor == 7) tabu_step_ended<L>(p.sa.state + (size_t)r * SA_WORDS, lane == 0, cur, applied ? &pick_sig : nullptr);
            if constexpr (!FAST)
                if (annealing) sa_step_ended(saw, p.sa, lane);
            wave_sync();
            st_steps += 1;
            if constexpr (SMALL) {
                st_gen += pulls;
                st_calc += pulls;
                st_acc += accepted;
                if constexpr (RBATCH) st_scored += pulls;
            }
            la_cursor = la_cursor + 1 >= la_size ? 0 : la_cursor + 1;
            const int64_t move_budget = SF_COLD_P(move_budget);
            if (move_budget > 0 && (int64_t)st_gen >= move_budget) {
                if constexpr (SMALL) ++step;
                break;
            }
            if (move_budget == 0 && st_scored >= 0x70000000u) flush_stats();
        }
        ISA_MARK("commit_end");
        PH(5)
    }
    PH_DUMP

    if (!dry_run) {
        if constexpr (!FAST)
            if (annealing) sa_store(saw, p.sa, r, lane);
        const uint32_t tot = uni(s_off[V]);
        uint32_t wlane = lane;
        SF_SPEC_OWN_LANE(wlane);
        const size_t n_cap = (size_t)SF_SPEC_NCAP(SF_COLD_M(n_cap));
        uint32_t* const w_visits = SMALL ? SF_COLD_M(visits) + (size_t)r * n_cap : g_visits;
        uint32_t* const w_off = SMALL ? SF_COLD_M(off) + (size_t)r * (V + 1) : g_off;
        int64_t* const w_load = SMALL ? SF_COLD_M(load) + (size_t)r * V : g_load;
        int64_t* const w_score = SMALL ? SF_COLD_M(score) + (size_t)r * 4 : g_score;
        if (best_pending) {
            uint32_t* const bv = SF_COLD_M(best_visits) + (size_t)r * n_cap;
            uint32_t* const bo = SF_COLD_M(best_off) + (size_t)r * (V + 1);
            for (uint32_t t = wlane; t < tot; t += 64) bv[t] = ext_id(s_visits[t]);
            for (uint32_t t = wlane; t <= (uint32_t)V; t += 64) bo[t] = s_off[t];
        }
        for (uint32_t t = wlane; t < tot; t += 64) w_visits[t] = ext_id(s_visits[t]);
        for (uint32_t t = wlane; t <= (uint32_t)V; t += 64) w_off[t] = s_off[t];
        for (uint32_t t = wlane; t < (uint32_t)V; t += 64) w_load[t] = (int64_t)s_load[t];
        if (lane == 0) {
#pragma unroll
            for (int kk = 0; kk < L; ++kk) {
                w_score[kk] = cur[kk];
                SF_COLD_P(last_step_score)[(size_t)r * 4 + kk] = cur[kk];
                SF_COLD_M(best_score)[(size_t)r * 4 + kk] = best_sol[kk];
            }
            SF_COLD_P(la_idx)[r] = la_cursor;
            const uint64_t ran = SMALL ? (uint64_t)step : steps_run + (uint64_t)st_steps;
            SF_COLD_P(step_index)[r] = step_index0 + ran;
            SF_COLD_P(seed_draws)[r] = seed_draws0 + ran;
        }
        flush_stats();
    }
    if (tracing && lane == 0) *p.trace_count = (int64_t)trace_n;
}

#undef SF_COLD_P
#undef SF_COLD_M

template <class F>
struct wave_args_are : std::false_type {};
template <>
struct wave_args_are<void (*)(decltype(WaveArgs::m), decltype(WaveArgs::p), decltype(WaveArgs::nb))> : std::true_type {};
static_assert(wave_args_are<decltype(&k_list_search_wave<2, false, 2>)>::value && std::is_standard_layout<WaveArgs>::value,
              "WaveArgs must list k_list_search_wave's parameters, in order: cold_args() reads the kernarg segment through it");

}
```

solverforge_amd/csrc/sf_tu_list_wave.hip:

```cpp
#define SF_TU_ENGINES 3
#include "sf_launch.h"

namespace sf {

template <>
hipError_t launch_tu_list_wave<SF_TU_L>(bool trace, int mode, const SearchLaunch& a) {
    if (mode == 6) return launch_with_lds(k_list_search_wave<SF_TU_L, false, 2, true, 4, true>, a, *a.lm, *a.p, a.nb);
    if (mode == 5) return launch_with_lds(k_list_search_wave<SF_TU_L, false, 2, true, 6>, a, *a.lm, *a.p, a.nb);
    if (mode == 4) return launch_with_lds(k_list_search_wave<SF_TU_L, false, 2, true, 5>, a, *a.lm, *a.p, a.nb);
    if (mode == 3) return launch_with_lds(k_list_search_wave<SF_TU_L, false, 2, true>, a, *a.lm, *a.p, a.nb);
    if (mode == 2) return launch_with_lds(k_list_search_wave<SF_TU_L, false, 2>, a, *a.lm, *a.p, a.nb);
    if (mode == 1) return launch_with_lds(k_list_search_wave<SF_TU_L, false, 1>, a, *a.lm, *a.p, a.nb);
    if (trace) return launch_with_lds(k_list_search_wave<SF_TU_L, true, 0>, a, *a.lm, *a.p, a.nb);
    return launch_with_lds(k_list_search_wave<SF_TU_L, false, 0>, a, *a.lm, *a.p, a.nb);
}

}

#if defined(SF_PHASE_PROFILE) || defined(SF_GEN_COUNT)
#define SF_PH_NAME2(l) sf_debug_phases_wave_##l
#define SF_PH_NAME(l) SF_PH_NAME2(l)
extern "C" int32_t SF_PH_NAME(SF_TU_L)(uint64_t* out8) {
    if (hipMemcpyFromSymbol(out8, HIP_SYMBOL(sf::g_phase), 64) != hipSuccess) return -1;
    unsigned long long z[8] = {0};
    (void)hipMemcpyToSymbol(HIP_SYMBOL(sf::g_phase), z, 64);
    return 0;
}
#endif
```

solverforge_amd/csrc/sf_wave_spec.h:

```cpp
#pragma once
#include <dlfcn.h>

#include "sf_nbr_facts.h"

#include <fstream>
#include <mutex>
#include <sstream>

struct WaveSpecKey {
    int32_t levels, wpe;
    int32_t V, dim, n_cap, k0, k1;
    int32_t extras;
    int32_t capacity, cap_weight, dist_weight, depot, cap_level, dist_level;
    int32_t la_size, limit, has_perm, has_explicit;
    int32_t wide_ties, ties, rows_full;
    int32_t index_x;
};
constexpr int32_t SF_WSPEC_KEY_WORDS_V1 = 18;
enum { SF_WSPEC_X_MODEL = 1, SF_WSPEC_X_LA = 2, SF_WSPEC_X_LIMIT = 4, SF_WSPEC_X_PERM = 8, SF_WSPEC_X_EXPLICIT = 16, SF_WSPEC_X_ALL = 31 };
enum { SF_WSPEC_X_NO_WIDE = 32, SF_WSPEC_X_TIE_KEY = 64, SF_WSPEC_X_NO_TIES = 128, SF_WSPEC_X_ROWS_FULL = 256, SF_WSPEC_X_INDEX_ALL = 480 };
constexpr int32_t SF_WSPEC_X_DEFAULT = SF_WSPEC_X_MODEL | SF_WSPEC_X_LA | SF_WSPEC_X_PERM;
constexpr int32_t SF_WSPEC_X_INDEX_DEFAULT = SF_WSPEC_X_NO_WIDE | SF_WSPEC_X_TIE_KEY | SF_WSPEC_X_ROWS_FULL;
static int32_t wave_spec_extras() {
    const char* e = std::getenv("SF_AMD_WAVE_SPEC_EXTRAS");
    return e ? (std::atoi(e) & (SF_WSPEC_X_ALL | SF_WSPEC_X_INDEX_ALL)) : (SF_WSPEC_X_DEFAULT | SF_WSPEC_X_INDEX_DEFAULT);
}

struct WaveSpecIndexGate {
    int32_t V, dim, n_cap;
    int32_t wide_ties, ties, rows_full;
};
static int32_t wave_spec_bits(uint32_t v) {
    int32_t b = 1;
    while (v >> b) ++b;
    return b;
}
static int32_t wave_spec_rb(int32_t V) { return wave_spec_bits((uint32_t)(V > 1 ? V - 1 : 0)); }
static int32_t wave_spec_pb(int32_t n_cap) { return wave_spec_bits((uint32_t)(n_cap > 0 ? n_cap : 0)); }
static int32_t wave_spec_index_allowed(const WaveSpecIndexGate& g) {
    int32_t a = 0;
    if (!g.wide_ties) a |= SF_WSPEC_X_NO_WIDE;
    if (wave_spec_rb(g.V) + wave_spec_pb(g.n_cap) <= 22) a |= SF_WSPEC_X_TIE_KEY;
    if (!g.ties) a |= SF_WSPEC_X_NO_TIES;
    if (g.rows_full && g.dim >= 32) a |= SF_WSPEC_X_ROWS_FULL;
    return a;
}
template <class Model, class Params>
static WaveSpecKey wave_spec_key(int32_t levels, int32_t wpe, const Model& m, const Params& q, const NbrFacts& nf, int32_t extras) {
    WaveSpecKey k{};
    k.levels = levels, k.wpe = wpe, k.V = m.V, k.dim = m.dim, k.n_cap = m.n_cap, k.k0 = q.leaf[0].max_nearby, k.k1 = q.leaf[1].max_nearby;
    k.wide_ties = nf.tie_max >= 64, k.ties = nf.tie_max >= 2, k.rows_full = nf.rows_full != 0;
    k.index_x = extras & SF_WSPEC_X_INDEX_ALL & wave_spec_index_allowed(WaveSpecIndexGate{k.V, k.dim, k.n_cap, k.wide_ties, k.ties, k.rows_full});
    extras &= SF_WSPEC_X_ALL;
    auto fits = [](int64_t v) { return v >= INT32_MIN && v <= INT32_MAX; };
    if ((extras & SF_WSPEC_X_MODEL) && !(fits(m.capacity) && fits(m.cap_weight) && fits(m.dist_weight))) extras &= ~SF_WSPEC_X_MODEL;
    if ((m.perm != nullptr) != (m.inv != nullptr)) extras &= ~SF_WSPEC_X_PERM;
    k.extras = extras;
    if (extras & SF_WSPEC_X_MODEL)
        k.capacity = (int32_t)m.capacity, k.cap_weight = (int32_t)m.cap_weight, k.dist_weight = (int32_t)m.dist_weight, k.depot = m.depot, k.cap_level = m.cap_level,
        k.dist_level = m.dist_level;
    if (extras & SF_WSPEC_X_LA) k.la_size = q.la_size;
    if (extras & SF_WSPEC_X_LIMIT) k.limit = q.limit;
    if (extras & SF_WSPEC_X_PERM) k.has_perm = m.perm != nullptr && m.inv != nullptr;
    if (extras & SF_WSPEC_X_EXPLICIT) k.has_explicit = q.explicit_seeds != nullptr;
    return k;
}
struct WaveSpecGate {
    int32_t mode, move_budget, n_steps;
    int32_t n_replicas, resident, cus;
    int32_t knob;
};
enum {
    SF_WSPEC_AOT = 0, SF_WSPEC_SPECIALISED = 1, SF_WSPEC_FELL_BACK = 2,
    SF_WSPEC_R_NONE = 0,
    SF_WSPEC_R_KNOB = 1, SF_WSPEC_R_MODE = 2, SF_WSPEC_R_BUDGET = 3, SF_WSPEC_R_STEPS = 4, SF_WSPEC_R_RESIDENCY = 5,
    SF_WSPEC_R_NO_HIPRTC = 10, SF_WSPEC_R_NO_SOURCES = 11, SF_WSPEC_R_COMPILE = 12, SF_WSPEC_R_LOAD = 13, SF_WSPEC_R_LDS = 14,
};
constexpr int32_t SF_WSPEC_MIN_STEPS = 50;

static int32_t wave_spec_wanted(const WaveSpecGate& g) {
    if (g.knob == 0) return SF_WSPEC_R_KNOB;
    if (g.mode < 3 || g.mode > 5) return SF_WSPEC_R_MODE;
    if (g.knob == 1) return SF_WSPEC_R_NONE;
    if (g.move_budget != 0) return SF_WSPEC_R_BUDGET;
    if (g.n_steps < SF_WSPEC_MIN_STEPS) return SF_WSPEC_R_STEPS;
    if ((int64_t)g.n_replicas < (int64_t)g.resident * g.cus) return SF_WSPEC_R_RESIDENCY;
    return SF_WSPEC_R_NONE;
}
static int32_t wave_spec_knob() {
    const char* e = std::getenv("SF_AMD_WAVE_SPEC");
    return e ? (std::atoi(e) != 0 ? 1 : 0) : -1;
}

static std::vector<std::string> wave_spec_options(const WaveSpecKey& k, const std::string& arch, const std::string& csrc, const std::string& rocm_include) {
    auto def = [](const char* name, int32_t v) { return std::string("-D") + name + "(x)=" + std::to_string(v); };
    std::vector<std::string> o{"--offload-arch=" + arch, "-O3", "-std=c++17", "-ffp-contract=off"};
    o.push_back("-I" + csrc);
    if (!rocm_include.empty()) o.push_back("-I" + rocm_include);
    o.push_back("-DSF_SPEC_L=" + std::to_string(k.levels));
    o.push_back("-DSF_SPEC_WPE=" + std::to_string(k.wpe));
    o.push_back(def("SF_SPEC_V", k.V));
    o.push_back(def("SF_SPEC_DIM", k.dim));
    o.push_back(def("SF_SPEC_NCAP", k.n_cap));
    o.push_back(def("SF_SPEC_K0", k.k0));
    o.push_back(def("SF_SPEC_K1", k.k1));
    auto word = [](const char* name, int32_t v) { return std::string("-D") + name + "=(" + std::to_string(v) + ")"; };
    if (k.extras & SF_WSPEC_X_MODEL)
        for (auto& x : {word("SF_SPEC_MODEL_WORDS", 1), word("SF_SPEC_CAPACITY", k.capacity), word("SF_SPEC_CAP_WEIGHT", k.cap_weight), word("SF_SPEC_DIST_WEIGHT", k.dist_weight),
                        word("SF_SPEC_DEPOT", k.depot), word("SF_SPEC_CAP_LEVEL", k.cap_level), word("SF_SPEC_DIST_LEVEL", k.dist_level)})
            o.push_back(x);
    if (k.extras & SF_WSPEC_X_LA) o.push_back(def("SF_SPEC_LA_SIZE", k.la_size));
    if (k.extras & SF_WSPEC_X_LIMIT) o.push_back(def("SF_SPEC_LIMIT", k.limit));
    if (k.extras & SF_WSPEC_X_PERM) o.push_back(def("SF_SPEC_HAS_PERM", k.has_perm));
    if (k.extras & SF_WSPEC_X_EXPLICIT) o.push_back(def("SF_SPEC_HAS_EXPLICIT", k.has_explicit));
    if (k.index_x & SF_WSPEC_X_NO_WIDE) o.push_back(word("SF_SPEC_NO_WIDE", 1));
    if (k.index_x & SF_WSPEC_X_TIE_KEY)
        for (auto& x : {word("SF_SPEC_TIE_KEY", 1), word("SF_SPEC_RB", wave_spec_rb(k.V)), word("SF_SPEC_PB", wave_spec_pb(k.n_cap))}) o.push_back(x);
    if (k.index_x & SF_WSPEC_X_NO_TIES) o.push_back(word("SF_SPEC_NO_TIES", 1));
    if (k.index_x & SF_WSPEC_X_ROWS_FULL) o.push_back(word("SF_SPEC_ROWS_FULL", 1));
    return o;
}
static std::string wave_spec_kernel_expr(const WaveSpecKey& k) {
    return "sf::k_list_search_wave<" + std::to_string(k.levels) + ", false, 2, true, " + std::to_string(k.wpe) + ", false>";
}
static bool wave_spec_key_ok(const WaveSpecKey& k) {
    return (k.levels == 2 || k.levels == 4) && k.wpe >= 4 && k.wpe <= 6 && k.V >= 1 && k.dim >= 1 && k.n_cap >= 0 && k.k0 >= 1 && k.k1 >= 1 && (k.extras & ~SF_WSPEC_X_ALL) == 0 &&
           (!(k.extras & SF_WSPEC_X_LA) || k.la_size >= 1) && (!(k.extras & SF_WSPEC_X_LIMIT) || k.limit >= 1) &&
           (k.wide_ties | k.ties | k.rows_full | 1) == 1 && (!k.wide_ties || k.ties) &&
           (k.index_x & ~wave_spec_index_allowed(WaveSpecIndexGate{k.V, k.dim, k.n_cap, k.wide_ties, k.ties, k.rows_full})) == 0;
}

struct WaveSpecRtc {
    void* lib = nullptr;
    std::string include_dir;
    int (*create)(void**, const char*, const char*, int, const char**, const char**) = nullptr;
    int (*compile)(void*, int, const char**) = nullptr;
    int (*destroy)(void**) = nullptr;
    int (*add_name)(void*, const char*) = nullptr;
    int (*lowered)(void*, const char*, const char**) = nullptr;
    int (*code_size)(void*, size_t*) = nullptr;
    int (*code)(void*, char*) = nullptr;
    int (*log_size)(void*, size_t*) = nullptr;
    int (*log)(void*, char*) = nullptr;
    bool ok() const { return lib && create && compile && destroy && add_name && lowered && code_size && code && log_size && log; }
};
static std::string wave_spec_dirname(const std::string& p) {
    const size_t s = p.find_last_of('/');
    return s == std::string::npos ? std::string(".") : p.substr(0, s);
}
static const WaveSpecRtc& wave_spec_rtc() {
    static const WaveSpecRtc once = [] {
        WaveSpecRtc r;
        for (const char* n : {"libhiprtc.so.7", "libhiprtc.so.6", "libhiprtc.so.5", "libhiprtc.so"})
            if ((r.lib = dlopen(n, RTLD_NOW | RTLD_LOCAL))) break;
        if (!r.lib) return r;
        auto sym = [&](const char* n) { return dlsym(r.lib, n); };
        r.create = (decltype(r.create))sym("hiprtcCreateProgram");
        r.compile = (decltype(r.compile))sym("hiprtcCompileProgram");
        r.destroy = (decltype(r.destroy))sym("hiprtcDestroyProgram");
        r.add_name = (decltype(r.add_name))sym("hiprtcAddNameExpression");
        r.lowered = (decltype(r.lowered))sym("hiprtcGetLoweredName");
        r.code_size = (decltype(r.code_size))sym("hiprtcGetCodeSize");
        r.code = (decltype(r.code))sym("hiprtcGetCode");
        r.log_size = (decltype(r.log_size))sym("hiprtcGetProgramLogSize");
        r.log = (decltype(r.log))sym("hiprtcGetProgramLog");
        Dl_info di;
        if (r.create && dladdr((void*)r.create, &di) && di.dli_fname) r.include_dir = wave_spec_dirname(wave_spec_dirname(di.dli_fname)) + "/include";
        return r;
    }();
    return once;
}
static std::string wave_spec_csrc() {
    if (const char* e = std::getenv("SF_AMD_CSRC")) return e;
    Dl_info di;
    if (dladdr((void*)&wave_spec_csrc, &di) && di.dli_fname) return wave_spec_dirname(di.dli_fname) + "/csrc";
    return "csrc";
}

struct WaveSpecBuild {
    int32_t reason = SF_WSPEC_R_NONE;
    std::vector<char> code;
    std::string kernel, log;
    double ms = 0;
};
static WaveSpecBuild wave_spec_compile(const WaveSpecKey& k, const std::string& arch, const std::string& csrc) {
    WaveSpecBuild b;
    const WaveSpecRtc& rtc = wave_spec_rtc();
    if (!rtc.ok()) return b.reason = SF_WSPEC_R_NO_HIPRTC, b;
    static const char* unit = "sf_tu_list_wave_spec.hip";
    std::ifstream f(csrc + "/" + unit, std::ios::binary);
    if (!f) return b.reason = SF_WSPEC_R_NO_SOURCES, b;
    std::stringstream src;
    src << f.rdbuf();
    const std::string text = src.str();
    const auto t0 = std::chrono::steady_clock::now();
    void* prog = nullptr;
    if (rtc.create(&prog, text.c_str(), unit, 0, nullptr, nullptr) != 0 || !prog) return b.reason = SF_WSPEC_R_COMPILE, b;
    const std::string expr = wave_spec_kernel_expr(k);
    const std::vector<std::string> opts = wave_spec_options(k, arch, csrc, rtc.include_dir);
    std::vector<const char*> argv;
    for (auto& o : opts) argv.push_back(o.c_str());
    int rc = rtc.add_name(prog, expr.c_str());
    if (rc == 0) rc = rtc.compile(prog, (int)argv.size(), argv.data());
    size_t n = 0;
    if (rtc.log_size(prog, &n) == 0 && n > 1) {
        b.log.resize(n);
        if (rtc.log(prog, &b.log[0]) != 0) b.log.clear();
    }
    const char* low = nullptr;
    if (rc == 0) rc = rtc.lowered(prog, expr.c_str(), &low);
    if (rc == 0 && low) b.kernel = low;
    if (rc == 0) rc = rtc.code_size(prog, &n);
    if (rc == 0) {
        b.code.resize(n);
        rc = rtc.code(prog, b.code.data());
    }
    (void)rtc.destroy(&prog);
    b.ms = std::chrono::duration<double, std::milli>(std::chrono::steady_clock::now() - t0).count();
    if (rc != 0 || b.kernel.empty() || b.code.empty()) b.reason = SF_WSPEC_R_COMPILE, b.code.clear();
    return b;
}

struct WaveSpecEntry {
    int32_t reason = SF_WSPEC_R_NONE;
    hipModule_t module = nullptr;
    hipFunction_t fn = nullptr;
    int lds_ok = 0;
};
struct WaveSpecCache {
    std::mutex mu;
    std::map<std::string, WaveSpecEntry> entries;
    int32_t compiles = 0;
    double last_ms = 0;
};
static WaveSpecCache& wave_spec_cache() {
    static WaveSpecCache c;
    return c;
}
static int32_t wave_spec_get(const WaveSpecKey& k, int device, size_t lds, hipFunction_t* fn) {
    WaveSpecCache& c = wave_spec_cache();
    const std::string csrc = wave_spec_csrc();
    std::string id = std::to_string(device) + "|" + csrc;
    const int32_t* w = &k.levels;
    for (size_t i = 0; i < sizeof(WaveSpecKey) / 4; ++i) id += "|" + std::to_string(w[i]);
    std::lock_guard<std::mutex> lock(c.mu);
    auto it = c.entries.find(id);
    if (it == c.entries.end()) {
        WaveSpecEntry e;
        hipDeviceProp_t prop;
        if (!wave_spec_key_ok(k) || hipGetDeviceProperties(&prop, device) != hipSuccess) {
            e.reason = SF_WSPEC_R_COMPILE;
        } else {
            std::string arch = prop.gcnArchName;
            arch = arch.substr(0, arch.find(':'));
            WaveSpecBuild b = wave_spec_compile(k, arch, csrc);
            if (b.reason != SF_WSPEC_R_NO_HIPRTC && b.reason != SF_WSPEC_R_NO_SOURCES) c.compiles += 1, c.last_ms = b.ms;
            e.reason = b.reason;
            if (!e.reason && (hipModuleLoadData(&e.module, b.code.data()) != hipSuccess || hipModuleGetFunction(&e.fn, e.module, b.kernel.c_str()) != hipSuccess)) {
                (void)hipGetLastError();
                e.reason = SF_WSPEC_R_LOAD, e.fn = nullptr;
            }
        }
        it = c.entries.emplace(id, e).first;
    }
    WaveSpecEntry& e = it->second;
    if (e.reason) return e.reason;
    if ((int)lds > e.lds_ok) {
        if (hipFuncSetAttribute((const void*)e.fn, hipFuncAttributeMaxDynamicSharedMemorySize, (int)lds) == hipSuccess) e.lds_ok = (int)lds;
        else {
            (void)hipGetLastError();
            if (lds > 64 * 1024) return SF_WSPEC_R_LDS;
        }
    }
    *fn = e.fn;
    return SF_WSPEC_R_NONE;
}
```

Measured before the change: 77.48 billion.

## Add symmetric lockstep fill/replay fast path when both leaves share K

Adds a lockstep mode, used when K0==K1<=32 under RBATCH, that generates pair batches for both leaves in unison into the rings, then replays full 64-lane batches (32 per leaf, interleaved by lane parity) without per-leaf bookkeeping. The pair generation and small replay bodies move into include files so the lockstep and general paths can share them. The aim is to drop per-iteration cursor management and partial-batch overhead in the fill/replay loop. It adds code size and register pressure, and falls back to the general path when either leaf emits fewer than K moves. An env knob can disable it.

```diff
diff --git a/solverforge_amd/csrc/sf_list_wave.hip b/solverforge_amd/csrc/sf_list_wave.hip
--- a/solverforge_amd/csrc/sf_list_wave.hip
+++ b/solverforge_amd/csrc/sf_list_wave.hip
@@ -532,8 +532,17 @@
     return emitted;
 }
 
+#ifndef SF_WAVE_SYM
+#define SF_WAVE_SYM 1
+#endif
+
 #if defined(SF_PHASE_PROFILE) || defined(SF_GEN_COUNT)
-__device__ unsigned long long g_phase[8];
+#ifdef SF_GEN_COUNT
+#define SF_PHASE_WORDS 10
+#else
+#define SF_PHASE_WORDS 8
+#endif
+__device__ unsigned long long g_phase[SF_PHASE_WORDS];
 #endif
 #ifdef SF_ISA_MARK
 #define ISA_MARK(name) asm volatile("; SF_MARK " name)
@@ -551,11 +560,11 @@
 #define PH_DUMP \
     if (lane == 0) for (int _k = 0; _k < 8; ++_k) atomicAdd(&g_phase[_k], (unsigned long long)ph_acc[_k]);
 #elif defined(SF_GEN_COUNT)
-#define PH_DECL uint64_t ph_acc[8] = {0, 0, 0, 0, 0, 0, 0, 0};
+#define PH_DECL uint64_t ph_acc[SF_PHASE_WORDS] = {0, 0, 0, 0, 0, 0, 0, 0, 0, 0};
 #define PH(i)
 #define GC(i) ph_acc[i] += 1;
 #define PH_DUMP \
-    if (lane == 0) for (int _k = 0; _k < 8; ++_k) atomicAdd(&g_phase[_k], (unsigned long long)ph_acc[_k]);
+    if (lane == 0) for (int _k = 0; _k < SF_PHASE_WORDS; ++_k) atomicAdd(&g_phase[_k], (unsigned long long)ph_acc[_k]);
 #else
 #define PH_DECL
 #define PH(i)
@@ -984,12 +993,23 @@
         const bool lane_hash = FAST && use_cm;
         if (lane_hash) {
             const uint64_t es0 = SALT_NEARBY_CHANGE_ENTITY ^ desc0(), es1 = SALT_NEARBY_SWAP_ENTITY ^ desc1();
-            const uint64_t salt = lane == 0 ? SALT_UNION_OFFSET : lane == 1 ? es0 : lane == 2 ? (es0 ^ STRIDE_SALT_MIX) : lane == 3 ? es1 : (es1 ^ STRIDE_SALT_MIX);
-            const FastMod fm2 = make_fastmod(2u);
-            FastMod f;
-            f.M = lane == 0 ? fm2.M : ((lane & 1u) ? fm_V.M : fm_V1.M);
-            f.n = lane == 0 ? fm2.n : ((lane & 1u) ? fm_V.n : fm_V1.n);
-            hashed = fastmod_u64(ctx.mixed_seed(salt), f);
+            if constexpr (RBATCH && SF_WAVE_SYM != 0) {
+                uint32_t hl = lane;
+                asm volatile("" : "+v"(hl));
+                const uint64_t salt = hl == 0 ? SALT_UNION_OFFSET : hl == 1 ? es0 : hl == 2 ? (es0 ^ STRIDE_SALT_MIX) : hl == 3 ? es1 : (es1 ^ STRIDE_SALT_MIX);
+                const FastMod fm2 = make_fastmod(2u);
+                FastMod f;
+                f.M = hl == 0 ? fm2.M : ((hl & 1u) ? fm_V.M : fm_V1.M);
+                f.n = hl == 0 ? fm2.n : ((hl & 1u) ? fm_V.n : fm_V1.n);
+                hashed = fastmod_u64(ctx.mixed_seed(salt), f);
+            } else {
+                const uint64_t salt = lane == 0 ? SALT_UNION_OFFSET : lane == 1 ? es0 : lane == 2 ? (es0 ^ STRIDE_SALT_MIX) : lane == 3 ? es1 : (es1 ^ STRIDE_SALT_MIX);
+                const FastMod fm2 = make_fastmod(2u);
+                FastMod f;
+                f.M = lane == 0 ? fm2.M : ((lane & 1u) ? fm_V.M : fm_V1.M);
+                f.n = lane == 0 ? fm2.n : ((lane & 1u) ? fm_V.n : fm_V1.n);
+                hashed = fastmod_u64(ctx.mixed_seed(salt), f);
+            }
         }
         const uint32_t first_leaf = lane_hash ? (uint32_t)__builtin_amdgcn_readlane((int)hashed, 0)
                                               : (n_leaves > 1 ? ctx.random_index((uint32_t)n_leaves, SALT_UNION_OFFSET) : 0u);
@@ -1121,6 +1141,8 @@
 
         PH(1)
         int done = 0;
+        constexpr bool SYM = RBATCH && SF_WAVE_SYM != 0;
+        [[maybe_unused]] bool lockstep = SYM && K0 == K1 && K0 <= 32u && total > 0;
         while (!done) {
             PH(4)
             auto gen_rest = [&](int l, uint32_t se, uint32_t sp, uint32_t len, uint32_t k, uint32_t sx, uint32_t tl,
@@ -1223,6 +1245,73 @@
                 } else
                     return node_slot.wide(word, node);
             };
+            if constexpr (SYM) {
+                if (lockstep) {
+                    lockstep = false;
+                    uint32_t sym_h = 0, sym_t = 0, sym_left = total, tA = 0, tB = 0;
+                    for (;;) {
+                        ISA_MARK("sym_fill_begin");
+                        bool leave = false;
+                        while (sym_t - sym_h < 32u) {
+                            tA = tB = sym_t;
+                            if (sym_left == 0) {
+                                leave = true;
+                                break;
+                            }
+                            ISA_MARK("pair_begin");
+                            GC(0)
+                            GC(8)
+                            uint32_t sym_left1 = sym_left;
+#define SF_PAIR_TAIL0 sym_t
+#define SF_PAIR_TAIL1 sym_t
+#define SF_PAIR_LEFT0 sym_left
+#define SF_PAIR_LEFT1 sym_left1
+#include "sf_wave_pair_pass.inc"
+#undef SF_PAIR_TAIL0
+#undef SF_PAIR_TAIL1
+#undef SF_PAIR_LEFT0
+#undef SF_PAIR_LEFT1
+                            ISA_MARK("pair_end");
+                            if (emA != K0 || emB != K0) {
+                                tA += emA;
+                                tB += emB;
+                                leave = true;
+                                break;
+                            }
+                            sym_t += K0;
+                        }
+                        ISA_MARK("sym_fill_end");
+                        if (leave) break;
+                        wave_sync();
+                        ISA_MARK("sym_replay_begin");
+                        {
+                            constexpr bool valid = true;
+                            constexpr uint32_t nvalid = 64u;
+                            uint32_t fl = first_leaf, ln = lane;
+                            asm volatile("" : "+s"(fl), "+v"(ln));
+                            const uint32_t lf = (fl + ln) & 1u, idx = sym_h + (ln >> 1);
+                            uint32_t m0, m1, nconsumed = nvalid;
+                            uint64_t accmask;
+                            [[maybe_unused]] bool doable, acc, consumed;
+#include "sf_wave_replay_small.inc"
+                            accepted += (uint32_t)__popcll(accmask);
+                            if (done) {
+                                pulls += nconsumed;
+                                break;
+                            }
+                        }
+                        sym_h += 32u;
+                        ISA_MARK("sym_replay_end");
+                    }
+                    pulls += 2u * sym_h;
+                    C0.head = C1.head = sym_h;
+                    C0.left = C1.left = sym_left;
+                    C0.tail = tA;
+                    C1.tail = tB;
+                    if (!done) { GC(9) }
+                    continue;
+                }
+            }
             const uint32_t single0 = cv.rc - K0 < 64u ? cv.rc - K0 : 64u, single1 = cv.rc - K1 < 64u ? cv.rc - K1 : 64u;
             ISA_MARK("fill_begin");
             for (;;) {
@@ -1233,179 +1322,15 @@
                 if (need0 && need1) {
                     ISA_MARK("pair_begin");
                     GC(0)
-                    const bool hi = lane >= 32;
-                    const uint32_t seA = C0.se, spA = C0.sp, lenA = C0.len, kA = C0.k, sxA = C0.sx, tlA = C0.tail;
-                    const uint32_t seB = C1.se, spB = C1.sp, lenB = C1.len, kB = C1.k, sxB = C1.sx, tlB = C1.tail;
-                    uint32_t l31 = lane & 31u;
-                    if constexpr (LEAN) asm volatile("" : "+v"(l31));
-                    const uint32_t key = LEAN ? (SF_SPEC_ROW_HAVE(false) ? half(C0.pk, C1.pk) : row_key(half(C0.pk, C1.pk), l31)) : (hi ? C1.pk : C0.pk);
-                    const bool have = SF_SPEC_ROW_HAVE(key != NBR_END);
-                    uint32_t nd = have ? (key & NBR_NODE_MASK) : 0u;
-                    uint32_t slot_word = 0;
-                    if constexpr (LEAN) {
-                        asm volatile("" : "+v"(nd)::"memory");
-                        slot_word = node_slot.word(nd);
-                    }
-                    C0.left -= 1;
-                    C0.o += 1;
-                    if (C0.left > 0) resolve(C0, 0);
-                    C1.left -= 1;
-                    C1.o += 1;
-                    if (C1.left > 0) resolve(C1, 1);
-                    if constexpr (!SMALL) st_sources += 2;
-                    uint32_t slot_any;
-                    if constexpr (LEAN)
-                        slot_any = slot_of(slot_word, nd);
-                    else
-                        slot_any = node_slot.get(nd);
-                    const uint32_t slot = have ? slot_any : NODE_NONE;
-                    NearbyItem it{0u, 0u, 0u, 0u};
-                    uint32_t mv0, tl, Kh, rq_off;
-                    if constexpr (LEAN) {
-                        const uint32_t sev = half(seA, seB), spv = half(spA, spB);
-                        mv0 = (sev << 16) | spv;
-                        tl = half(tlA, tlB);
-                        Kh = half(K0, K1);
-                        rq_off = hm & (cv.rc * 2u);
-                        const bool some = slot != NODE_NONE;
-                        const uint32_t r_any = slot >> 16, dp = slot & 0xFFFFu;
-                        const uint32_t r2 = some ? r_any : 0u;
-                        const uint32_t len2 = s_off[r2 + 1] - s_off[r2];
-                        uint32_t t;
-                        if constexpr (ARANK)
-                            t = RouteArith{half(perm_st0, perm_st1), half(perm_inv0, perm_inv1), (uint32_t)V, v_recip32}.word(r2);
-                        else
-                            t = rtab[r2 + (hm & (uint32_t)V)];
-                        const bool intra = r2 == sev;
-                        const uint32_t end_pay = (r2 << 16) | len2;
-                        const uint32_t xi = dp - (spv & ~hm), yi = half(1u, spv);
-                        const uint32_t xo = RT::rank(t) | ~hm, yo = kB & hm;
-                        const uint32_t xs = intra ? xi : xo, ys = intra ? yi : yo;
-                        const bool v0 = xs > ys;
-                        const uint32_t last = lenA ^ (spv + 1u);
-                        const uint32_t f = intra ? last : 1u;
-                        const uint32_t z1 = (((dp + 1u) ^ len2) | hm) | (1u - min(f, 1u));
-                        const bool v1 = z1 == 0u;
-                        const uint32_t b0 = v0 ? 1u : 0u, b1 = v1 ? 1u : 0u;
-                        const uint32_t wsum = b0 + b1;
-                        it.w = some ? wsum : 0u;
-                        const uint32_t len_or_dp = half(lenA, dp), ord_intra = v0 ? dp : len_or_dp, ord_inter = RT::inter_ord(t, dp);
-                        it.ord = intra ? ord_intra : ord_inter;
-                        const uint32_t end_or_slot = half(end_pay, slot);
-                        it.pay0 = v0 ? slot : end_or_slot;
-                        it.pay1 = end_pay;
-                    } else {
-                        const uint32_t se = hi ? seB : seA, sp = hi ? spB : spA, len = hi ? lenB : lenA, kk = hi ? kB : kA;
-                        mv0 = (se << 16) | sp;
-                        tl = hi ? tlB : tlA;
-                        Kh = hi ? K1 : K0;
-                        rq_off = hi ? cv.rc * 2u : 0u;
-                        RT rth;
-                        if constexpr (ARANK)
-                            rth = RouteArith{hi ? perm_st1 : perm_st0, hi ? perm_inv1 : perm_inv0, (uint32_t)V, v_recip32};
-                        else
-                            rth = RT{rtab + (hi ? V : 0)};
-                        if constexpr (FAST) {
-                            const bool some = slot != NODE_NONE;
-                            const uint32_t r2 = some ? slot >> 16 : 0u, dp = slot & 0xFFFFu;
-                            const uint32_t len2 = s_off[r2 + 1] - s_off[r2];
-                            const uint32_t t = rth.word(r2);
-                            const bool intra = r2 == se;
-                            const uint32_t end_pay = (r2 << 16) | len2;
-                            const bool v0 = hi ? (intra ? dp > sp : RT::rank(t) > kk) : (!intra || dp - sp >= 2u);
-                            const bool v1 = !hi && dp + 1 == len2 && (!intra || len != sp + 1);
-                            it.w = some ? (uint32_t)v0 + (uint32_t)v1 : 0u;
-                            it.ord = intra ? ((hi || v0) ? dp : len) : RT::inter_ord(t, dp);
-                            it.pay0 = (hi || v0) ? slot : end_pay;
-                            it.pay1 = end_pay;
-                        } else {
-                            const NearbyItem ic = nearby_item_rt(true, slot, se, sp, len, kk, s_off, rth);
-                            const NearbyItem is = nearby_item_rt(false, slot, se, sp, len, kk, s_off, rth);
-                            const bool lane_change = hi ? chg1 : chg0;
-                            it.w = lane_change ? ic.w : is.w;
-                            it.ord = lane_change ? ic.ord : is.ord;
-                            it.pay0 = lane_change ? ic.pay0 : is.pay0;
-                            it.pay1 = lane_change ? ic.pay1 : is.pay1;
-                        }
-                    }
-                    const uint64_t havemask = SF_SPEC_ROW_HAVEMASK(__ballot(have));
-                    const uint64_t startmask = LEAN ? __ballot(key < NBR_END - min(l31, 1u) * (NBR_END - NBR_SAME_FLAG))
-                                                        : __ballot(have && (l31 == 0 || !(key & NBR_SAME_FLAG)));
-                    const uint32_t hvA = (uint32_t)havemask, hvB = (uint32_t)(havemask >> 32);
-                    const uint32_t stA = (uint32_t)startmask, stB = (uint32_t)(startmask >> 32);
-                    const bool moreA = hvA == 0xFFFFFFFFu && 32u < dim, moreB = hvB == 0xFFFFFFFFu && 32u < dim;
-                    uint32_t ncA = 0, ncB = 0;
-                    uint64_t closedmask;
-                    bool closed;
-                    if constexpr (LEAN) {
-                        const uint32_t hvv = half(hvA, hvB), stv = half(stA, stB);
-                        const uint32_t ncv = (hvv == 0xFFFFFFFFu && 32u < dim) ? 31u - (uint32_t)__clz(stv) : (uint32_t)__popc(hvv);
-                        closed = l31 < ncv;
-                        closedmask = __ballot(closed);
-                    } else {
-                        ncA = moreA ? 31u - (uint32_t)__clz(stA) : (uint32_t)__popc(hvA);
-                        ncB = moreB ? 31u - (uint32_t)__clz(stB) : (uint32_t)__popc(hvB);
-                        closedmask = (uint64_t)(ncA >= 32 ? 0xFFFFFFFFu : ((1u << ncA) - 1u)) |
-                                     ((uint64_t)(ncB >= 32 ? 0xFFFFFFFFu : ((1u << ncB) - 1u)) << 32);
-                        closed = (closedmask & lanebit) != 0;
-                    }
-                    const uint32_t wc = closed ? it.w : 0u;
-                    const uint64_t w1 = __ballot(wc == 1), w2 = __ballot(wc == 2);
-                    const uint32_t WcA = (uint32_t)__popc((uint32_t)w1) + 2u * (uint32_t)__popc((uint32_t)w2);
-                    const uint32_t WcB = (uint32_t)__popc((uint32_t)(w1 >> 32)) + 2u * (uint32_t)__popc((uint32_t)(w2 >> 32));
-                    if (WcA + WcB > 0) {
-                        const uint32_t pa = __builtin_amdgcn_mbcnt_lo((uint32_t)w1, 0u) + 2u * __builtin_amdgcn_mbcnt_lo((uint32_t)w2, 0u);
-                        const uint32_t pb = __builtin_amdgcn_mbcnt_hi((uint32_t)(w1 >> 32), 0u) + 2u * __builtin_amdgcn_mbcnt_hi((uint32_t)(w2 >> 32), 0u);
-                        int32_t pos = (int32_t)(LEAN ? half(pa, pb) : (hi ? pb : pa));
-                        const uint64_t nonstart = SF_SPEC_TIES(~startmask & closedmask);
-#ifdef SF_SPEC_TIE_KEY
-                        static_assert(!std::is_same<RT, RouteTab>::value, "SF_SPEC_TIE_KEY: the (rank, position) ordinals");
-                        if (nonstart) pos += tie_key_fix(startmask, nonstart, it.ord, wc);
-#else
-                        if (nonstart) {
-                            const uint32_t packed = (it.ord << 2) | wc;
-                            uint64_t run = nonstart;
-                            uint32_t p_dn = packed, p_up = packed;
-                            for (uint32_t d = 1; run != 0; ++d) {
-                                p_dn = (uint32_t)__builtin_amdgcn_update_dpp(0, (int)p_dn, 0x130, 0xf, 0xf, false);
-                                p_up = (uint32_t)__builtin_amdgcn_update_dpp(0, (int)p_up, 0x138, 0xf, 0xf, false);
-                                const bool same_up = (run & lanebit) != 0;
-                                const bool same_dn = ((run >> d) & lanebit) != 0;
-                                if (same_dn && (p_dn >> 2) < it.ord) pos += (int32_t)(p_dn & 3u);
-                                if (same_up && (p_up >> 2) > it.ord) pos -= (int32_t)(p_up & 3u);
-                                run &= nonstart << d;
-                            }
-                        }
-#endif
-                        uint32_t* rq = ring + rq_off;
-                        if (wc >= 1 && (uint32_t)pos < Kh) {
-                            const uint32_t qi = (tl + (uint32_t)pos) & RCM;
-                            rq[qi * 2] = mv0;
-                            rq[qi * 2 + 1] = it.pay0;
-                        }
-                        if (wc == 2 && (uint32_t)pos + 1 < Kh) {
-                            const uint32_t qi = (tl + (uint32_t)pos + 1) & RCM;
-                            rq[qi * 2] = mv0;
-                            rq[qi * 2 + 1] = it.pay1;
-                        }
-                    }
-                    uint32_t emA = WcA < K0 ? WcA : K0, emB = WcB < K1 ? WcB : K1;
-                    if (emA < K0 && moreA) {
-                        GC(3)
-                        ISA_MARK("pair_rest_begin");
-                        if constexpr (LEAN) ncA = 31u - (uint32_t)__clz(stA);
-                        const uint32_t jj = ncA + lane;
-                        emA = gen_rest(0, seA, spA, lenA, kA, sxA, tlA, jj < dim ? (uint32_t)nb.keys[(size_t)sxA * dim + jj] : NBR_END, ncA, K0 - emA, emA);
-                        ISA_MARK("pair_rest_end");
-                    }
-                    if (emB < K1 && moreB) {
-                        GC(4)
-                        ISA_MARK("pair_rest_begin");
-                        if constexpr (LEAN) ncB = 31u - (uint32_t)__clz(stB);
-                        const uint32_t jj = ncB + lane;
-                        emB = gen_rest(1, seB, spB, lenB, kB, sxB, tlB, jj < dim ? (uint32_t)nb.keys[(size_t)sxB * dim + jj] : NBR_END, ncB, K1 - emB, emB);
-                        ISA_MARK("pair_rest_end");
-                    }
+#define SF_PAIR_TAIL0 C0.tail
+#define SF_PAIR_TAIL1 C1.tail
+#define SF_PAIR_LEFT0 C0.left
+#define SF_PAIR_LEFT1 C1.left
+#include "sf_wave_pair_pass.inc"
+#undef SF_PAIR_TAIL0
+#undef SF_PAIR_TAIL1
+#undef SF_PAIR_LEFT0
+#undef SF_PAIR_LEFT1
                     C0.tail = tlA + emA;
                     C1.tail = tlB + emB;
                     ISA_MARK("pair_end");
@@ -1468,88 +1393,7 @@
                 uint64_t accmask = 0;
                 uint32_t nconsumed = nvalid;
                 if constexpr (SMALL) {
-                    int32_t dv[L];
-                    {
-                        const uint32_t lf0 = (uint32_t)__builtin_amdgcn_readfirstlane((int)lf), idx0 = (uint32_t)__builtin_amdgcn_readfirstlane((int)idx);
-                        const uint32_t lfq = valid ? lf : lf0;
-                        const uint32_t qi = (valid ? idx : idx0) & RCM;
-                        const uint32_t* rq = ring + ((size_t)lfq * cv.rc + qi) * 2;
-                        m0 = rq[0];
-                        m1 = rq[1];
-                        const uint32_t a = m0 >> 16, i = m0 & 0xFFFFu, b = m1 >> 16, j = m1 & 0xFFFFu;
-                        eval_generated_small<L, LT, COMPACT, OT, RBATCH>(m, lvl, s_visits, s_off, s_load, 1u - lfq, a, i, b, j, dv);
-                    }
-                    doable = valid;
-                    int64_t key = 0;
-                    if constexpr (L == 2) {
-                        key = (int64_t)(((uint64_t)(uint32_t)dv[0] << 32) + (uint64_t)(int64_t)dv[1]);
-                        acc = valid && key >= acc_thr;
-                    } else {
-                        acc = valid && (small_ge0<L>(dv) || small_ge<L>(dv, late_d));
-                    }
-                    accmask = __ballot(acc);
-                    consumed = valid;
-                    if (!RBATCH || (uint32_t)__popcll(accmask) >= (uint32_t)SF_SPEC_LIMIT(p.limit) - accepted) {
-                        const uint32_t remaining = (uint32_t)SF_SPEC_LIMIT(p.limit) - accepted;
-                        const uint32_t pre = mbcnt64(accmask) + (acc ? 1u : 0u);
-                        const uint64_t cutmask = __ballot(acc && pre == remaining);
-                        nconsumed = cutmask ? (uint32_t)__ffsll((unsigned long long)cutmask) : nvalid;
-                        consumed = lane < nconsumed;
-                        acc = acc && consumed;
-                        accmask = __ballot(acc);
-                        if constexpr (RBATCH) {
-                            st_scored += nvalid - nconsumed;
-                            done = 1;
-                        }
-                    }
-                    bool challenger;
-                    if constexpr (L == 2)
-                        challenger = acc && key >= best_key;
-                    else
-                        challenger = acc && small_ge<L>(dv, best_d);
-                    if (accmask && (!has_best || __ballot(challenger))) {
-                        int32_t M[L];
-                        bool in_max = acc;
-#pragma unroll
-                        for (int kk = 0; kk < L; ++kk) {
-                            M[kk] = wave_max_i32(in_max ? dv[kk] : (int32_t)0x80000000);
-                            in_max = in_max && dv[kk] == M[kk];
-                        }
-                        int64_t Mkey = 0;
-                        if constexpr (L == 2) Mkey = (int64_t)(((uint64_t)(uint32_t)M[0] << 32) + (uint64_t)(int64_t)M[1]);
-                        bool ge, gt;
-                        if constexpr (L == 2) {
-                            ge = !has_best || Mkey >= best_key;
-                            gt = !has_best || Mkey > best_key;
-                        } else {
-                            ge = !has_best || small_ge<L>(M, best_d);
-                            gt = !has_best || !small_ge<L>(best_d, M);
-                        }
-                        if (ge) {
-                            const bool newmax = gt;
-                            const uint32_t eq_base = newmax ? 0u : equal_count;
-                            const uint64_t eq = __ballot(in_max);
-                            const uint32_t rank = mbcnt64(eq) + 1u;
-                            const uint64_t cntq = (uint64_t)(eq_base + rank);
-                            const bool pick = in_max && ((newmax && rank == 1) ||
-                                                         (p.random_ties && cntq > 1 && reservoir_pick(sseed, cntq)));
-                            const uint64_t pm = __ballot(pick);
-                            if (pm) {
-                                const int sel = 63 - __clzll((unsigned long long)pm);
-                                best_m0 = __shfl(m0, sel);
-                                best_m1 = __shfl(m1, sel);
-                                best_leaf = (int)__shfl(lf, sel);
-                            }
-                            if constexpr (L == 2) {
-                                best_key = Mkey;
-                            } else {
-#pragma unroll
-                                for (int kk = 0; kk < L; ++kk) best_d[kk] = M[kk];
-                            }
-                            equal_count = eq_base + (uint32_t)__popcll(eq);
-                            has_best = 1;
-                        }
-                    }
+#include "sf_wave_replay_small.inc"
                 } else {
                     ListDelta dl{0, 0, false};
                     if (valid) {
diff --git a/solverforge_amd/csrc/sf_tu_list_wave.hip b/solverforge_amd/csrc/sf_tu_list_wave.hip
--- a/solverforge_amd/csrc/sf_tu_list_wave.hip
+++ b/solverforge_amd/csrc/sf_tu_list_wave.hip
@@ -20,10 +20,10 @@
 #if defined(SF_PHASE_PROFILE) || defined(SF_GEN_COUNT)
 #define SF_PH_NAME2(l) sf_debug_phases_wave_##l
 #define SF_PH_NAME(l) SF_PH_NAME2(l)
-extern "C" int32_t SF_PH_NAME(SF_TU_L)(uint64_t* out8) {
-    if (hipMemcpyFromSymbol(out8, HIP_SYMBOL(sf::g_phase), 64) != hipSuccess) return -1;
-    unsigned long long z[8] = {0};
-    (void)hipMemcpyToSymbol(HIP_SYMBOL(sf::g_phase), z, 64);
+extern "C" int32_t SF_PH_NAME(SF_TU_L)(uint64_t* out) {
+    if (hipMemcpyFromSymbol(out, HIP_SYMBOL(sf::g_phase), sizeof(sf::g_phase)) != hipSuccess) return -1;
+    unsigned long long z[SF_PHASE_WORDS] = {0};
+    (void)hipMemcpyToSymbol(HIP_SYMBOL(sf::g_phase), z, sizeof(z));
     return 0;
 }
 #endif
diff --git a/solverforge_amd/csrc/sf_wave_pair_pass.inc b/solverforge_amd/csrc/sf_wave_pair_pass.inc
--- /dev/null
+++ b/solverforge_amd/csrc/sf_wave_pair_pass.inc
@@ -0,0 +1,173 @@
+const bool hi = lane >= 32;
+const uint32_t seA = C0.se, spA = C0.sp, lenA = C0.len, kA = C0.k, sxA = C0.sx, tlA = SF_PAIR_TAIL0;
+const uint32_t seB = C1.se, spB = C1.sp, lenB = C1.len, kB = C1.k, sxB = C1.sx, tlB = SF_PAIR_TAIL1;
+uint32_t l31 = lane & 31u;
+if constexpr (LEAN) asm volatile("" : "+v"(l31));
+const uint32_t key = LEAN ? (SF_SPEC_ROW_HAVE(false) ? half(C0.pk, C1.pk) : row_key(half(C0.pk, C1.pk), l31)) : (hi ? C1.pk : C0.pk);
+const bool have = SF_SPEC_ROW_HAVE(key != NBR_END);
+uint32_t nd = have ? (key & NBR_NODE_MASK) : 0u;
+uint32_t slot_word = 0;
+if constexpr (LEAN) {
+    asm volatile("" : "+v"(nd)::"memory");
+    slot_word = node_slot.word(nd);
+}
+SF_PAIR_LEFT0 -= 1;
+C0.o += 1;
+if (SF_PAIR_LEFT0 > 0) resolve(C0, 0);
+SF_PAIR_LEFT1 -= 1;
+C1.o += 1;
+if (SF_PAIR_LEFT1 > 0) resolve(C1, 1);
+if constexpr (!SMALL) st_sources += 2;
+uint32_t slot_any;
+if constexpr (LEAN)
+    slot_any = slot_of(slot_word, nd);
+else
+    slot_any = node_slot.get(nd);
+const uint32_t slot = have ? slot_any : NODE_NONE;
+NearbyItem it{0u, 0u, 0u, 0u};
+uint32_t mv0, tl, Kh, rq_off;
+if constexpr (LEAN) {
+    const uint32_t sev = half(seA, seB), spv = half(spA, spB);
+    mv0 = (sev << 16) | spv;
+    tl = half(tlA, tlB);
+    Kh = half(K0, K1);
+    rq_off = hm & (cv.rc * 2u);
+    const bool some = slot != NODE_NONE;
+    const uint32_t r_any = slot >> 16, dp = slot & 0xFFFFu;
+    const uint32_t r2 = some ? r_any : 0u;
+    const uint32_t len2 = s_off[r2 + 1] - s_off[r2];
+    uint32_t t;
+    if constexpr (ARANK)
+        t = RouteArith{half(perm_st0, perm_st1), half(perm_inv0, perm_inv1), (uint32_t)V, v_recip32}.word(r2);
+    else
+        t = rtab[r2 + (hm & (uint32_t)V)];
+    const bool intra = r2 == sev;
+    const uint32_t end_pay = (r2 << 16) | len2;
+    const uint32_t xi = dp - (spv & ~hm), yi = half(1u, spv);
+    const uint32_t xo = RT::rank(t) | ~hm, yo = kB & hm;
+    const uint32_t xs = intra ? xi : xo, ys = intra ? yi : yo;
+    const bool v0 = xs > ys;
+    const uint32_t last = lenA ^ (spv + 1u);
+    const uint32_t f = intra ? last : 1u;
+    const uint32_t z1 = (((dp + 1u) ^ len2) | hm) | (1u - min(f, 1u));
+    const bool v1 = z1 == 0u;
+    const uint32_t b0 = v0 ? 1u : 0u, b1 = v1 ? 1u : 0u;
+    const uint32_t wsum = b0 + b1;
+    it.w = some ? wsum : 0u;
+    const uint32_t len_or_dp = half(lenA, dp), ord_intra = v0 ? dp : len_or_dp, ord_inter = RT::inter_ord(t, dp);
+    it.ord = intra ? ord_intra : ord_inter;
+    const uint32_t end_or_slot = half(end_pay, slot);
+    it.pay0 = v0 ? slot : end_or_slot;
+    it.pay1 = end_pay;
+} else {
+    const uint32_t se = hi ? seB : seA, sp = hi ? spB : spA, len = hi ? lenB : lenA, kk = hi ? kB : kA;
+    mv0 = (se << 16) | sp;
+    tl = hi ? tlB : tlA;
+    Kh = hi ? K1 : K0;
+    rq_off = hi ? cv.rc * 2u : 0u;
+    RT rth;
+    if constexpr (ARANK)
+        rth = RouteArith{hi ? perm_st1 : perm_st0, hi ? perm_inv1 : perm_inv0, (uint32_t)V, v_recip32};
+    else
+        rth = RT{rtab + (hi ? V : 0)};
+    if constexpr (FAST) {
+        const bool some = slot != NODE_NONE;
+        const uint32_t r2 = some ? slot >> 16 : 0u, dp = slot & 0xFFFFu;
+        const uint32_t len2 = s_off[r2 + 1] - s_off[r2];
+        const uint32_t t = rth.word(r2);
+        const bool intra = r2 == se;
+        const uint32_t end_pay = (r2 << 16) | len2;
+        const bool v0 = hi ? (intra ? dp > sp : RT::rank(t) > kk) : (!intra || dp - sp >= 2u);
+        const bool v1 = !hi && dp + 1 == len2 && (!intra || len != sp + 1);
+        it.w = some ? (uint32_t)v0 + (uint32_t)v1 : 0u;
+        it.ord = intra ? ((hi || v0) ? dp : len) : RT::inter_ord(t, dp);
+        it.pay0 = (hi || v0) ? slot : end_pay;
+        it.pay1 = end_pay;
+    } else {
+        const NearbyItem ic = nearby_item_rt(true, slot, se, sp, len, kk, s_off, rth);
+        const NearbyItem is = nearby_item_rt(false, slot, se, sp, len, kk, s_off, rth);
+        const bool lane_change = hi ? chg1 : chg0;
+        it.w = lane_change ? ic.w : is.w;
+        it.ord = lane_change ? ic.ord : is.ord;
+        it.pay0 = lane_change ? ic.pay0 : is.pay0;
+        it.pay1 = lane_change ? ic.pay1 : is.pay1;
+    }
+}
+const uint64_t havemask = SF_SPEC_ROW_HAVEMASK(__ballot(have));
+const uint64_t startmask = LEAN ? __ballot(key < NBR_END - min(l31, 1u) * (NBR_END - NBR_SAME_FLAG))
+                                    : __ballot(have && (l31 == 0 || !(key & NBR_SAME_FLAG)));
+const uint32_t hvA = (uint32_t)havemask, hvB = (uint32_t)(havemask >> 32);
+const uint32_t stA = (uint32_t)startmask, stB = (uint32_t)(startmask >> 32);
+const bool moreA = hvA == 0xFFFFFFFFu && 32u < dim, moreB = hvB == 0xFFFFFFFFu && 32u < dim;
+uint32_t ncA = 0, ncB = 0;
+uint64_t closedmask;
+bool closed;
+if constexpr (LEAN) {
+    const uint32_t hvv = half(hvA, hvB), stv = half(stA, stB);
+    const uint32_t ncv = (hvv == 0xFFFFFFFFu && 32u < dim) ? 31u - (uint32_t)__clz(stv) : (uint32_t)__popc(hvv);
+    closed = l31 < ncv;
+    closedmask = __ballot(closed);
+} else {
+    ncA = moreA ? 31u - (uint32_t)__clz(stA) : (uint32_t)__popc(hvA);
+    ncB = moreB ? 31u - (uint32_t)__clz(stB) : (uint32_t)__popc(hvB);
+    closedmask = (uint64_t)(ncA >= 32 ? 0xFFFFFFFFu : ((1u << ncA) - 1u)) |
+                 ((uint64_t)(ncB >= 32 ? 0xFFFFFFFFu : ((1u << ncB) - 1u)) << 32);
+    closed = (closedmask & lanebit) != 0;
+}
+const uint32_t wc = closed ? it.w : 0u;
+const uint64_t w1 = __ballot(wc == 1), w2 = __ballot(wc == 2);
+const uint32_t WcA = (uint32_t)__popc((uint32_t)w1) + 2u * (uint32_t)__popc((uint32_t)w2);
+const uint32_t WcB = (uint32_t)__popc((uint32_t)(w1 >> 32)) + 2u * (uint32_t)__popc((uint32_t)(w2 >> 32));
+if (WcA + WcB > 0) {
+    const uint32_t pa = __builtin_amdgcn_mbcnt_lo((uint32_t)w1, 0u) + 2u * __builtin_amdgcn_mbcnt_lo((uint32_t)w2, 0u);
+    const uint32_t pb = __builtin_amdgcn_mbcnt_hi((uint32_t)(w1 >> 32), 0u) + 2u * __builtin_amdgcn_mbcnt_hi((uint32_t)(w2 >> 32), 0u);
+    int32_t pos = (int32_t)(LEAN ? half(pa, pb) : (hi ? pb : pa));
+    const uint64_t nonstart = SF_SPEC_TIES(~startmask & closedmask);
+#ifdef SF_SPEC_TIE_KEY
+    static_assert(!std::is_same<RT, RouteTab>::value, "SF_SPEC_TIE_KEY: the (rank, position) ordinals");
+    if (nonstart) pos += tie_key_fix(startmask, nonstart, it.ord, wc);
+#else
+    if (nonstart) {
+        const uint32_t packed = (it.ord << 2) | wc;
+        uint64_t run = nonstart;
+        uint32_t p_dn = packed, p_up = packed;
+        for (uint32_t d = 1; run != 0; ++d) {
+            p_dn = (uint32_t)__builtin_amdgcn_update_dpp(0, (int)p_dn, 0x130, 0xf, 0xf, false);
+            p_up = (uint32_t)__builtin_amdgcn_update_dpp(0, (int)p_up, 0x138, 0xf, 0xf, false);
+            const bool same_up = (run & lanebit) != 0;
+            const bool same_dn = ((run >> d) & lanebit) != 0;
+            if (same_dn && (p_dn >> 2) < it.ord) pos += (int32_t)(p_dn & 3u);
+            if (same_up && (p_up >> 2) > it.ord) pos -= (int32_t)(p_up & 3u);
+            run &= nonstart << d;
+        }
+    }
+#endif
+    uint32_t* rq = ring + rq_off;
+    if (wc >= 1 && (uint32_t)pos < Kh) {
+        const uint32_t qi = (tl + (uint32_t)pos) & RCM;
+        rq[qi * 2] = mv0;
+        rq[qi * 2 + 1] = it.pay0;
+    }
+    if (wc == 2 && (uint32_t)pos + 1 < Kh) {
+        const uint32_t qi = (tl + (uint32_t)pos + 1) & RCM;
+        rq[qi * 2] = mv0;
+        rq[qi * 2 + 1] = it.pay1;
+    }
+}
+uint32_t emA = WcA < K0 ? WcA : K0, emB = WcB < K1 ? WcB : K1;
+if (emA < K0 && moreA) {
+    GC(3)
+    ISA_MARK("pair_rest_begin");
+    if constexpr (LEAN) ncA = 31u - (uint32_t)__clz(stA);
+    const uint32_t jj = ncA + lane;
+    emA = gen_rest(0, seA, spA, lenA, kA, sxA, tlA, jj < dim ? (uint32_t)nb.keys[(size_t)sxA * dim + jj] : NBR_END, ncA, K0 - emA, emA);
+    ISA_MARK("pair_rest_end");
+}
+if (emB < K1 && moreB) {
+    GC(4)
+    ISA_MARK("pair_rest_begin");
+    if constexpr (LEAN) ncB = 31u - (uint32_t)__clz(stB);
+    const uint32_t jj = ncB + lane;
+    emB = gen_rest(1, seB, spB, lenB, kB, sxB, tlB, jj < dim ? (uint32_t)nb.keys[(size_t)sxB * dim + jj] : NBR_END, ncB, K1 - emB, emB);
+    ISA_MARK("pair_rest_end");
+}
diff --git a/solverforge_amd/csrc/sf_wave_replay_small.inc b/solverforge_amd/csrc/sf_wave_replay_small.inc
--- /dev/null
+++ b/solverforge_amd/csrc/sf_wave_replay_small.inc
@@ -0,0 +1,82 @@
+int32_t dv[L];
+{
+    const uint32_t lf0 = (uint32_t)__builtin_amdgcn_readfirstlane((int)lf), idx0 = (uint32_t)__builtin_amdgcn_readfirstlane((int)idx);
+    const uint32_t lfq = valid ? lf : lf0;
+    const uint32_t qi = (valid ? idx : idx0) & RCM;
+    const uint32_t* rq = ring + ((size_t)lfq * cv.rc + qi) * 2;
+    m0 = rq[0];
+    m1 = rq[1];
+    const uint32_t a = m0 >> 16, i = m0 & 0xFFFFu, b = m1 >> 16, j = m1 & 0xFFFFu;
+    eval_generated_small<L, LT, COMPACT, OT, RBATCH>(m, lvl, s_visits, s_off, s_load, 1u - lfq, a, i, b, j, dv);
+}
+doable = valid;
+int64_t key = 0;
+if constexpr (L == 2) {
+    key = (int64_t)(((uint64_t)(uint32_t)dv[0] << 32) + (uint64_t)(int64_t)dv[1]);
+    acc = valid && key >= acc_thr;
+} else {
+    acc = valid && (small_ge0<L>(dv) || small_ge<L>(dv, late_d));
+}
+accmask = __ballot(acc);
+consumed = valid;
+if (!RBATCH || (uint32_t)__popcll(accmask) >= (uint32_t)SF_SPEC_LIMIT(p.limit) - accepted) {
+    const uint32_t remaining = (uint32_t)SF_SPEC_LIMIT(p.limit) - accepted;
+    const uint32_t pre = mbcnt64(accmask) + (acc ? 1u : 0u);
+    const uint64_t cutmask = __ballot(acc && pre == remaining);
+    nconsumed = cutmask ? (uint32_t)__ffsll((unsigned long long)cutmask) : nvalid;
+    consumed = lane < nconsumed;
+    acc = acc && consumed;
+    accmask = __ballot(acc);
+    if constexpr (RBATCH) {
+        st_scored += nvalid - nconsumed;
+        done = 1;
+    }
+}
+bool challenger;
+if constexpr (L == 2)
+    challenger = acc && key >= best_key;
+else
+    challenger = acc && small_ge<L>(dv, best_d);
+if (accmask && (!has_best || __ballot(challenger))) {
+    int32_t M[L];
+    bool in_max = acc;
+#pragma unroll
+    for (int kk = 0; kk < L; ++kk) {
+        M[kk] = wave_max_i32(in_max ? dv[kk] : (int32_t)0x80000000);
+        in_max = in_max && dv[kk] == M[kk];
+    }
+    int64_t Mkey = 0;
+    if constexpr (L == 2) Mkey = (int64_t)(((uint64_t)(uint32_t)M[0] << 32) + (uint64_t)(int64_t)M[1]);
+    bool ge, gt;
+    if constexpr (L == 2) {
+        ge = !has_best || Mkey >= best_key;
+        gt = !has_best || Mkey > best_key;
+    } else {
+        ge = !has_best || small_ge<L>(M, best_d);
+        gt = !has_best || !small_ge<L>(best_d, M);
+    }
+    if (ge) {
+        const bool newmax = gt;
+        const uint32_t eq_base = newmax ? 0u : equal_count;
+        const uint64_t eq = __ballot(in_max);
+        const uint32_t rank = mbcnt64(eq) + 1u;
+        const uint64_t cntq = (uint64_t)(eq_base + rank);
+        const bool pick = in_max && ((newmax && rank == 1) ||
+                                     (p.random_ties && cntq > 1 && reservoir_pick(sseed, cntq)));
+        const uint64_t pm = __ballot(pick);
+        if (pm) {
+            const int sel = 63 - __clzll((unsigned long long)pm);
+            best_m0 = __shfl(m0, sel);
+            best_m1 = __shfl(m1, sel);
+            best_leaf = (int)__shfl(lf, sel);
+        }
+        if constexpr (L == 2) {
+            best_key = Mkey;
+        } else {
+#pragma unroll
+            for (int kk = 0; kk < L; ++kk) best_d[kk] = M[kk];
+        }
+        equal_count = eq_base + (uint32_t)__popcll(eq);
+        has_best = 1;
+    }
+}
diff --git a/solverforge_amd/csrc/sf_wave_spec.h b/solverforge_amd/csrc/sf_wave_spec.h
--- a/solverforge_amd/csrc/sf_wave_spec.h
+++ b/solverforge_amd/csrc/sf_wave_spec.h
@@ -90,6 +90,11 @@
 static int32_t wave_spec_knob() {
     const char* e = std::getenv("SF_AMD_WAVE_SPEC");
     return e ? (std::atoi(e) != 0 ? 1 : 0) : -1;
+}
+
+static bool wave_spec_no_sym() {
+    static const bool once = std::getenv("SF_AMD_NO_WAVE_SYM") != nullptr;
+    return once;
 }
 
 static std::vector<std::string> wave_spec_options(const WaveSpecKey& k, const std::string& arch, const std::string& csrc, const std::string& rocm_include) {
@@ -118,6 +123,7 @@
         for (auto& x : {word("SF_SPEC_TIE_KEY", 1), word("SF_SPEC_RB", wave_spec_rb(k.V)), word("SF_SPEC_PB", wave_spec_pb(k.n_cap))}) o.push_back(x);
     if (k.index_x & SF_WSPEC_X_NO_TIES) o.push_back(word("SF_SPEC_NO_TIES", 1));
     if (k.index_x & SF_WSPEC_X_ROWS_FULL) o.push_back(word("SF_SPEC_ROWS_FULL", 1));
+    if (wave_spec_no_sym()) o.push_back("-DSF_WAVE_SYM=0");
     return o;
 }
 static std::string wave_spec_kernel_expr(const WaveSpecKey& k) {
```

New measurement: 85.17 billion, median of 6. +9.9%, better.
